# ViktorNfa/bluerov2_dynamics

Hardware: AMD Instinct MI355X
Metric: rk4_rollout_steps_per_s (higher is better)
Workload: dtype f64; 1 GPU; BASELINE config 2: 65536 trajectories/GPU x 5000 RK4 steps, thruster model, dt=0.02, iid U(-1,1) commands (splitmix64 stream 0x5EED), layout tpb, all states stored; trajectories_per_gpu=65536, horizon=5000, parallelism=1 x independent shards, no collective

## Files before the change

bluerov2_dynamics_amd/_lib.py:

```python
import ctypes
import os
import threading

import numpy as np

from . import _build

c_double_p = ctypes.POINTER(ctypes.c_double)
c_void_p = ctypes.c_void_p
i64 = ctypes.c_int64

THRUSTER_EULER, WRENCH_EULER, WRENCH_QUAT = 0, 1, 2
DI_THRUSTER_EULER, DI_WRENCH_EULER, DI_WRENCH_QUAT = 3, 4, 5
EULER, RK4 = 0, 1
LAG_PER_CALL, LAG_PER_STEP = 0, 1
LAYOUT_BTU, LAYOUT_TUB, LAYOUT_TPB = 0, 1, 2
DIST_IID_UNIFORM, DIST_AR1 = 0, 1
NX = {THRUSTER_EULER: 12, WRENCH_EULER: 12, WRENCH_QUAT: 13, DI_THRUSTER_EULER: 12, DI_WRENCH_EULER: 12, DI_WRENCH_QUAT: 13}
NU = {THRUSTER_EULER: 8, WRENCH_EULER: 6, WRENCH_QUAT: 6, DI_THRUSTER_EULER: 8, DI_WRENCH_EULER: 6, DI_WRENCH_QUAT: 6}
STATUS = {0: "BROV_OK", -1: "BROV_ERR_ARG", -2: "BROV_ERR_HIP", -3: "BROV_ERR_NOMEM", -4: "BROV_ERR_NODEVICE", -5: "BROV_ERR_COMM"}
COMM_ID_BYTES = 128


class BrovParams(ctypes.Structure):
# ... 160 lines not shown
                                       ctypes.POINTER(BrovUkf), i64, i64, ctypes.c_double] + [c_void_p] * 16 + [i64]),
    "brov_ukf_smooth_dev": (ctypes.c_int, [c_void_p, ctypes.c_int, ctypes.c_int, ctypes.c_int, i64, ctypes.POINTER(BrovParams), i64,
                                           ctypes.POINTER(BrovUkf), i64, i64, ctypes.c_double] + [c_void_p] * 16 + [i64]),
    "brov_mppi_step": (ctypes.c_int, [c_void_p, ctypes.c_int, ctypes.c_int, ctypes.c_int, i64, i64, ctypes.POINTER(BrovParams),
                                      ctypes.POINTER(BrovMppi), i64, i64, ctypes.c_double, ctypes.c_uint64, c_void_p, c_void_p, c_void_p,
                                      i64, i64, c_void_p, c_void_p, ctypes.c_int, c_void_p, c_void_p, c_void_p]),
    "brov_mppi_step_dev": (ctypes.c_int, [c_void_p, ctypes.c_int, ctypes.c_int, ctypes.c_int, i64, i64, ctypes.POINTER(BrovParams),
                                          ctypes.POINTER(BrovMppi), i64, i64, ctypes.c_double, ctypes.c_uint64, c_void_p, c_void_p,
                                          c_void_p, i64, i64, c_void_p, c_void_p, ctypes.c_int, c_void_p, c_void_p, c_void_p]),
    "edmdc_mppi_step": (ctypes.c_int, [c_void_p, ctypes.c_int, ctypes.c_int, ctypes.c_int, ctypes.c_double, c_void_p, c_void_p, c_void_p, c_void_p,
                                       c_void_p, i64, ctypes.POINTER(BrovMppi), i64, i64, ctypes.c_double, ctypes.c_uint64, c_void_p, c_void_p,
                                       i64, i64, c_void_p, c_void_p, ctypes.c_int, c_void_p, c_void_p, c_void_p, c_void_p]),
    "edmdc_mppi_step_dev": (ctypes.c_int, [c_void_p, ctypes.c_int, ctypes.c_int, ctypes.c_int, ctypes.c_double, c_void_p, c_void_p, c_void_p,
                                           c_void_p, c_void_p, i64, ctypes.POINTER(BrovMppi), i64, i64, ctypes.c_double, ctypes.c_uint64,
                                           c_void_p, c_void_p, i64, i64, c_void_p, c_void_p, ctypes.c_int, c_void_p, c_void_p, c_void_p,
                                           c_void_p]),
    "edmdc_lmpc_step": (ctypes.c_int, [c_void_p, ctypes.c_int, ctypes.c_int, ctypes.c_int, ctypes.c_double] + [c_void_p] * 6 +
                        [i64, ctypes.POINTER(BrovLmpc), i64, ctypes.c_double, c_void_p, c_void_p, i64, i64, c_void_p, c_void_p, ctypes.c_int,
                         c_void_p, c_void_p, c_void_p]),
    "edmdc_lmpc_step_dev": (ctypes.c_int, [c_void_p, ctypes.c_int, ctypes.c_int, ctypes.c_int, ctypes.c_double] + [c_void_p] * 6 +
                            [i64, ctypes.POINTER(BrovLmpc), i64, ctypes.c_double, c_void_p, c_void_p, i64, i64, c_void_p, c_void_p,
                             ctypes.c_int, c_void_p, c_void_p, c_void_p]),
    "edmdc_lmpc_block_lds": (ctypes.c_int, [i64, ctypes.POINTER(ctypes.c_int)]),
    "brov_pinc_set_weights": (ctypes.c_int, [c_void_p, c_void_p, i64]),
    "brov_pinc_forward_dev": (ctypes.c_int, [c_void_p, i64, c_void_p, c_void_p]),
    "brov_pinc_rollout": (ctypes.c_int, [c_void_p, i64, i64, ctypes.c_double, c_void_p, c_void_p, c_void_p, c_void_p, i64, c_void_p]),
    "brov_pinc_rollout_dev": (ctypes.c_int, [c_void_p, i64, i64, ctypes.c_double, c_void_p, c_void_p, c_void_p, c_void_p, i64, c_void_p]),
    "brov_pinc_window_endpoint_se": (ctypes.c_int, [c_void_p, i64, i64, ctypes.c_double, c_void_p, c_void_p, ctypes.c_int, c_void_p,
                                                    c_void_p, c_void_p, c_void_p]),
    "brov_pinc_window_endpoint_se_dev": (ctypes.c_int, [c_void_p, i64, i64, ctypes.c_double, c_void_p, c_void_p, ctypes.c_int, c_void_p,
                                                        c_void_p, c_void_p, c_void_p]),
    "brov_pinc_loss_grad_dev": (ctypes.c_int, [c_void_p, c_void_p, i64, c_void_p, c_void_p, c_void_p, ctypes.c_int, ctypes.c_int,
                                               c_void_p, c_void_p]),
    "brov_pinc_adamw_step_dev": (ctypes.c_int, [c_void_p, c_void_p, c_void_p, c_void_p, c_void_p, i64] + [ctypes.c_double] * 6 + [c_void_p]),
    "brov_pinc_train_begin": (ctypes.c_int, [c_void_p, c_void_p, i64, ctypes.POINTER(PincHyper)]),
    "brov_pinc_train_set_state": (ctypes.c_int, [c_void_p, c_void_p, c_void_p, i64]),
    "brov_pinc_train_epoch_dev": (ctypes.c_int, [c_void_p, i64, c_void_p, c_void_p, c_void_p, c_void_p, c_void_p]),
    "brov_pinc_train_get": (ctypes.c_int, [c_void_p, c_void_p, c_void_p, c_void_p, ctypes.POINTER(i64)]),
    "brov_pinc_train_end": (ctypes.c_int, [c_void_p]),
    "brov_thruster_stream": (ctypes.c_int, [c_void_p, i64, c_void_p, ctypes.c_double, c_void_p, c_void_p]),
    "brov_thruster_stream_dev": (ctypes.c_int, [c_void_p, i64, c_void_p, ctypes.c_double, c_void_p, c_void_p]),
    "brov_fill_controls_dev": (ctypes.c_int, [c_void_p, ctypes.c_int, ctypes.c_int, i64, i64, ctypes.c_int,
                                              ctypes.c_uint64, i64, i64, c_void_p, c_void_p]),
    "edmdc_lift": (ctypes.c_int, [c_void_p, i64, ctypes.c_int, ctypes.c_int, ctypes.c_double, c_void_p, c_void_p, c_void_p]),
    "edmdc_gram": (ctypes.c_int, [c_void_p, ctypes.c_int, ctypes.c_int, ctypes.c_int, ctypes.c_double, c_void_p,
                                  i64, i64, i64, i64, c_void_p, c_void_p, ctypes.c_int, c_void_p, c_void_p]),
    "edmdc_gram_dev": (ctypes.c_int, [c_void_p, ctypes.c_int, ctypes.c_int, ctypes.c_int, ctypes.c_double, c_void_p,
                                      i64, i64, i64, i64, c_void_p, c_void_p, ctypes.c_int, c_void_p, c_void_p]),
    "edmdc_gram_ragged": (ctypes.c_int, [c_void_p, ctypes.c_int, ctypes.c_int, ctypes.c_int, ctypes.c_double, c_void_p,
                                         i64, c_void_p, c_void_p, c_void_p, ctypes.c_int, c_void_p, c_void_p]),
    "edmdc_gram_ragged_dev": (ctypes.c_int, [c_void_p, ctypes.c_int, ctypes.c_int, ctypes.c_int, ctypes.c_double, c_void_p,
                                             i64, c_void_p, c_void_p, c_void_p, ctypes.c_int, c_void_p, c_void_p]),
    "edmdc_pinv_apply_ragged": (ctypes.c_int, [c_void_p, ctypes.c_int, ctypes.c_int, ctypes.c_int, ctypes.c_double, c_void_p,
                                               i64, c_void_p, c_void_p, c_void_p, c_void_p, c_void_p]),
    "edmdc_pinv_apply_ragged_dev": (ctypes.c_int, [c_void_p, ctypes.c_int, ctypes.c_int, ctypes.c_int, ctypes.c_double, c_void_p,
                                                   i64, c_void_p, c_void_p, c_void_p, c_void_p, c_void_p]),
    "brov_upload_bags": (ctypes.c_int, [c_void_p, i64, c_void_p, c_void_p, c_void_p, ctypes.c_int, c_void_p]),
    "edmdc_set_chunk_rows": (ctypes.c_int, [c_void_p, i64]),
    "edmdc_kmeans_lloyd": (ctypes.c_int, [c_void_p, i64, ctypes.c_int, ctypes.c_int, c_void_p, c_void_p, c_void_p, ctypes.c_int,
                                          ctypes.c_double, c_void_p, ctypes.POINTER(ctypes.c_double), ctypes.POINTER(ctypes.c_int)]),
    "edmdc_kmeans_lloyd_dev": (ctypes.c_int, [c_void_p, i64, ctypes.c_int, ctypes.c_int, c_void_p, i64, c_void_p, c_void_p, ctypes.c_int,
                                              ctypes.c_double, c_void_p, ctypes.POINTER(ctypes.c_double), ctypes.POINTER(ctypes.c_int)]),
    "edmdc_kmeanspp_dev": (ctypes.c_int, [c_void_p, i64, ctypes.c_int, ctypes.c_int, c_void_p, i64, c_void_p, i64, ctypes.c_int, c_void_p,
                                          c_void_p, c_void_p]),
    "edmdc_multistep_se": (ctypes.c_int, [c_void_p, ctypes.c_int, ctypes.c_int, ctypes.c_int, ctypes.c_double, c_void_p,
                                          c_void_p, c_void_p, i64, i64, c_void_p, c_void_p, c_void_p, c_void_p]),
    "edmdc_multistep_se_linear": (ctypes.c_int, [c_void_p, ctypes.c_int, ctypes.c_int, ctypes.c_int, ctypes.c_double, c_void_p,
                                                 c_void_p, c_void_p, i64, i64, c_void_p, c_void_p, c_void_p, c_void_p]),
    "edmdc_simulate": (ctypes.c_int, [c_void_p, ctypes.c_int, ctypes.c_int, ctypes.c_int, ctypes.c_double, c_void_p,
                                      c_void_p, c_void_p, i64, i64, c_void_p, c_void_p, c_void_p]),
    "edmdc_pinv_apply": (ctypes.c_int, [c_void_p, ctypes.c_int, ctypes.c_int, ctypes.c_int, ctypes.c_double, c_void_p,
                                        i64, i64, i64, i64, c_void_p, c_void_p, c_void_p, c_void_p]),
    "edmdc_pinv_apply_dev": (ctypes.c_int, [c_void_p, ctypes.c_int, ctypes.c_int, ctypes.c_int, ctypes.c_double, c_void_p,
                                            i64, i64, i64, i64, c_void_p, c_void_p, c_void_p, c_void_p]),
    "edmdc_gram_decomposition": (ctypes.c_int, [ctypes.c_int, ctypes.c_int, ctypes.c_int, ctypes.POINTER(ctypes.c_int), ctypes.POINTER(ctypes.c_int)]),
    "edmdc_gtg_decomposition": (ctypes.c_int, [ctypes.c_int, ctypes.c_int, ctypes.c_int, ctypes.POINTER(ctypes.c_int), ctypes.POINTER(ctypes.c_int)]),
    "edmdc_apply_decomposition": (ctypes.c_int, [ctypes.c_int, ctypes.c_int, ctypes.c_int] + [ctypes.POINTER(ctypes.c_int)] * 4),
    "edmdc_set_apply_variant": (ctypes.c_int, [c_void_p, ctypes.c_int]),
    "edmdc_lift_cache": (ctypes.c_int, [c_void_p, c_void_p, ctypes.c_size_t]),
    "edmdc_set_kmeans_variant": (ctypes.c_int, [c_void_p, ctypes.c_int]),
    "edmdc_set_kmeans_bounds_rate": (ctypes.c_int, [c_void_p, ctypes.c_double]),
    "brov_experiments_build": (ctypes.c_int, []),
    "brov_set_rollout_variant": (ctypes.c_int, [c_void_p, ctypes.c_int]),
    "edmdc_set_kmeans_far_select": (ctypes.c_int, [c_void_p, c_void_p, c_void_p]),
    "edmdc_kmeans_relocations": (ctypes.c_int, [c_void_p]),
    "edmdc_kmeans_loop_info": (ctypes.c_int, [c_void_p, ctypes.POINTER(ctypes.c_int)]),
    "edmdc_far_select_numpy": (ctypes.c_int, [c_void_p, i64, ctypes.c_int, c_void_p]),
    "edmdc_set_kmeans_allreduce": (ctypes.c_int, [c_void_p, c_void_p, c_void_p]),
    "edmdc_set_kmeans_shard": (ctypes.c_int, [c_void_p, ctypes.c_int, ctypes.c_int, i64, i64]),
    "brov_comm_available": (ctypes.c_int, []),
    "brov_comm_unique_id": (ctypes.c_int, [c_void_p]),
    "brov_comm_init_rank": (ctypes.c_int, [ctypes.c_int, c_void_p, ctypes.c_int, ctypes.c_int, ctypes.POINTER(c_void_p)]),
    "brov_comm_destroy": (None, [c_void_p]),
    "brov_comm_nranks": (ctypes.c_int, [c_void_p]),
    "brov_comm_rank": (ctypes.c_int, [c_void_p]),
    "brov_comm_last_error": (ctypes.c_char_p, [c_void_p]),
    "edmdc_gram_allreduce_dev": (ctypes.c_int, [c_void_p, c_void_p, i64, c_void_p, i64, c_void_p]),
    "brov_comm_allreduce_words": (ctypes.c_int, [c_void_p, c_void_p, i64, ctypes.c_int, c_void_p]),
    "edmdc_kmeans_use_comm": (ctypes.c_int, [c_void_p, c_void_p]),
}


def library_path():
    return _build.LIB


hip_runtime = None


def _one_hip_runtime():
    import sys
    if "torch" in sys.modules:
        return "torch (imported by the caller)"
    mode = os.environ.get("BROV2_TORCH", "auto").strip().lower()
    if mode in ("1", "import", "yes", "true"):
        try:
            import torch
            return "torch (imported by load_library: BROV2_TORCH=1)"
        except ImportError:
            return "system (BROV2_TORCH=1 but torch is not installed)"
    if mode in ("0", "no", "never", "false"):
        return "system (BROV2_TORCH=0)"
    try:
        import importlib.util
        spec = importlib.util.find_spec("torch")
    except (ImportError, ValueError):
        spec = None
    if spec is not None and spec.origin:
        cand = os.path.join(os.path.dirname(spec.origin), "lib", "libamdhip64.so")
        if os.path.exists(cand):
            try:
                ctypes.CDLL(cand, mode=ctypes.RTLD_GLOBAL)
                return "torch's libamdhip64.so preloaded (torch itself not imported)"
            except OSError:
                pass
    return "system"


def load_library():
    global _lib, hip_runtime
    with _lib_lock:
        if _lib is not None:
            return _lib
        path = library_path()
        if not os.path.exists(path):
            raise BrovError(
                f"{path} is missing: build it with `python -c 'import __graft_entry__ as g; g.build()'` "
                "(hipcc --offload-arch=gfx950). There is no CPU fallback.")
        hip_runtime = _one_hip_runtime()
        lib = ctypes.CDLL(path)
        for name, (res, args) in SIGNATURES.items():
            fn = getattr(lib, name)
            fn.restype = res
            fn.argtypes = args
        if lib.brov_abi_version() != 1:
            raise BrovError("libbrov2.so ABI version mismatch")
        _lib = lib
        return lib


def default_params() -> BrovParams:
    p = BrovParams()
    load_library().brov_default_params(ctypes.byref(p))
    return p


# ... 33 lines not shown

class Context:

    def __init__(self, device: int = 0):
        self.lib = load_library()
        h = c_void_p()
        rc = self.lib.brov_create(int(device), ctypes.byref(h))
        if rc != 0:
            raise BrovError(f"brov_create(device={device}) failed: {STATUS.get(rc, rc)} -- a gfx950 GPU is required, "
                            "there is no CPU fallback")
        self.h = h
        self.device = int(device)
        self._stream = 0
        self._allreduce_cb = None
        self.check(self.lib.edmdc_set_kmeans_far_select(self.h, ctypes.cast(_NUMPY_FAR_SELECT, c_void_p), None), "edmdc_set_kmeans_far_select")

    @property
    def arch(self) -> str:
        buf = ctypes.create_string_buffer(64)
        self.check(self.lib.brov_device_arch(self.h, buf, 64), "brov_device_arch")
        return buf.value.decode()

    @property
    def xcd_round_robin(self) -> int:
        return int(self.lib.brov_xcd_round_robin(self.h))

    def close(self):
        if getattr(self, "h", None):
            self.lib.brov_destroy(self.h)
            self.h = None

    def __del__(self):
        try:
            self.close()
        except Exception:
            pass

    def check(self, rc, what=""):
        if rc != 0:
            msg = self.lib.brov_last_error(self.h)
            raise BrovError(f"{what}: {STATUS.get(rc, rc)}: {msg.decode() if msg else ''}")

    def get_params(self) -> BrovParams:
        p = BrovParams()
        self.check(self.lib.brov_get_params(self.h, ctypes.byref(p)), "brov_get_params")
        return p

    def set_params(self, p: BrovParams):
        self.check(self.lib.brov_set_params(self.h, ctypes.byref(p)), "brov_set_params")

    def set_stream(self, stream_handle):
        stream_handle = int(stream_handle or 0)
        if stream_handle != self._stream:
            self.check(self.lib.brov_set_stream(self.h, c_void_p(stream_handle)), "brov_set_stream")
            self._stream = stream_handle

    def use_torch_stream(self):
        import torch
        self.set_stream(torch.cuda.current_stream(self.device).cuda_stream)

    def use_null_stream(self):
        self.set_stream(0)

    def set_di_gains(self, K_lin, K_ang):
        K_lin, K_ang = as_f64(K_lin), as_f64(K_ang)
        assert K_lin.shape == K_ang.shape and K_lin.shape[1] == 3
        self.check(self.lib.brov_set_di_gains(self.h, int(K_lin.shape[0]), K_lin.ctypes.data, K_ang.ctypes.data), "brov_set_di_gains")

    def set_btu_staging(self, mode: int):
        self.check(self.lib.brov_set_btu_staging(self.h, int(mode)), "brov_set_btu_staging")

    def lift_cache(self, device_ptr, nbytes: int = 0):
        self.check(self.lib.edmdc_lift_cache(self.h, c_void_p(device_ptr or 0), int(nbytes if device_ptr else 0)), "edmdc_lift_cache")

    def set_kmeans_variant(self, variant: int):
        self.check(self.lib.edmdc_set_kmeans_variant(self.h, int(variant)), "edmdc_set_kmeans_variant")

    def set_kmeans_bounds_rate(self, rate: float):
        self.check(self.lib.edmdc_set_kmeans_bounds_rate(self.h, float(rate)), "edmdc_set_kmeans_bounds_rate")

    def set_rollout_variant(self, variant: int):
        self.check(self.lib.brov_set_rollout_variant(self.h, int(variant)), "brov_set_rollout_variant")

    def set_kmeans_far_select(self, numpy_rule: bool):
        fn = ctypes.cast(_NUMPY_FAR_SELECT, c_void_p) if numpy_rule else None
        self.check(self.lib.edmdc_set_kmeans_far_select(self.h, fn, None), "edmdc_set_kmeans_far_select")

    def kmeans_relocations(self) -> int:
        return int(self.lib.edmdc_kmeans_relocations(self.h))

    def kmeans_loop_info(self) -> dict:
        v = (ctypes.c_int * 4)()
        self.check(self.lib.edmdc_kmeans_loop_info(self.h, v), "edmdc_kmeans_loop_info")
        return dict(relocations=v[0], resorts=v[1], first_resort_iteration=v[2], list_form_e_steps=v[3])

    def set_kmeans_allreduce(self, fn):
        if fn is None:
            self._allreduce_cb = None
            self.check(self.lib.edmdc_set_kmeans_allreduce(self.h, None, None), "edmdc_set_kmeans_allreduce")
            return

        def tramp(_user, ptr, count, op):
            try:
                fn(int(ptr), int(count), int(op))
                return 0
            except Exception:
                import traceback
                traceback.print_exc()
                return 1
        self._allreduce_cb = ALLREDUCE_FN(tramp)
        self.check(self.lib.edmdc_set_kmeans_allreduce(self.h, ctypes.cast(self._allreduce_cb, c_void_p), None), "edmdc_set_kmeans_allreduce")

    def set_kmeans_shard(self, rank: int = 0, world: int = 1, row_offset: int = 0, n_global: int = 0):
        self.check(self.lib.edmdc_set_kmeans_shard(self.h, int(rank), int(world), int(row_offset), int(n_global)), "edmdc_set_kmeans_shard")

    def kmeans_use_comm(self, comm):
        self.check(self.lib.edmdc_kmeans_use_comm(self.h, comm.h if comm is not None else None), "edmdc_kmeans_use_comm")

    def set_apply_variant(self, variant: int):
        self.check(self.lib.edmdc_set_apply_variant(self.h, int(variant)), "edmdc_set_apply_variant")

    def sync(self):
        self.check(self.lib.brov_sync(self.h), "brov_sync")

    def set_timing(self, on: bool):
        self.check(self.lib.brov_set_timing(self.h, int(bool(on))), "brov_set_timing")
        self.timing = bool(on)

    def last_kernel_ms(self) -> float:
        ms = ctypes.c_float(0.0)
        self.check(self.lib.brov_last_kernel_ms(self.h, ctypes.byref(ms)), "brov_last_kernel_ms")
        return float(ms.value)


_default = {}
_default_lock = threading.Lock()


def default_context(device: int = None) -> Context:
    if device is None:
        device = int(os.environ.get("BROV2_DEVICE", os.environ.get("LOCAL_RANK", "0")))
    ctx = _default.get(device)
    if ctx is None:
        with _default_lock:
            ctx = _default.get(device)
            if ctx is None:
                ctx = _default[device] = Context(device)
    return ctx


def warm_up(device: int = None, block: bool = False):
    def work():
        try:
            default_context(device)
        except Exception:
            pass
    if block:
        return default_context(device)
    t = threading.Thread(target=work, name="brov2-warm-up", daemon=True)
    t.start()
    return t


class Comm:

    def __init__(self, device: int, unique_id: bytes, nranks: int, rank: int):
# ... 48 lines not shown
```

bluerov2_dynamics_amd/csrc/brov2_fast.h:

```cpp
#pragma once
#include "brov2_device.h"

namespace brov {

struct FastParams {
    double E[12];
    double da[6], db[6];
    double G[5];
    double lc[4][3];
    double ld[4];
    double Tm[6][8];
    double minv[6];
    double poly[5];
    double A1[9], b1[3];
    double A4[9], b4[3];
    double Ob[9];
    double al4[3];
    double Aw4[9], bw4[3];
    double g1[3];
    double XY[4];
    double cur[3];
    int has_current;
    int has_xy;
    int tm_dense;
    int obs_bad;
};

typedef const FastParams __attribute__((address_space(4)))* CFP;
__device__ __forceinline__ CFP as_constant(const FastParams* g) { return (CFP)(unsigned long long)g; }

template <bool RES>
struct HotConstsT {
    static constexpr bool RESIDENT = RES;
    double E[12], db[6];
    double da[6], G[5], ld[4], al4[3];
    double tk[2];
};
typedef HotConstsT<false> HotConsts;
typedef HotConstsT<true> HotConstsResident;

#ifndef BROV_CLAMP_BRANCH
#define BROV_CLAMP_BRANCH 1
#endif
#ifndef BROV_PSI_FRAME
#define BROV_PSI_FRAME 1
#endif
#define BROV_PIN_V(x) asm volatile("" : "+v"(x))
#define BROV_PIN_S(x) asm volatile("" : "+s"(x))
#define BROV_FORM_HERE(r) asm volatile("" : "+v"(r))
#define BROV_SC(h, p, f) (HC::RESIDENT ? (h).f : (p)->f)

template <bool RES>
__device__ __forceinline__ void load_hot(CFP pp, HotConstsT<RES>& h) {
    const auto& p = *pp;
#pragma unroll
    for (int i = 0; i < 12; ++i) { h.E[i] = p.E[i]; BROV_PIN_V(h.E[i]); }
#pragma unroll
    for (int i = 0; i < 6; ++i) { h.db[i] = p.db[i]; BROV_PIN_V(h.db[i]); }
    if constexpr (RES) {
#pragma unroll
        for (int i = 0; i < 6; ++i) { h.da[i] = p.da[i]; BROV_PIN_S(h.da[i]); }
#pragma unroll
        for (int i = 0; i < 5; ++i) { h.G[i] = p.G[i]; BROV_PIN_S(h.G[i]); }
#pragma unroll
        for (int i = 0; i < 4; ++i) { h.ld[i] = p.ld[i]; BROV_PIN_S(h.ld[i]); }
#pragma unroll
        for (int i = 0; i < 3; ++i) { h.al4[i] = p.al4[i]; BROV_PIN_S(h.al4[i]); }
        h.tk[0] = -1.98412698298579493134e-04; BROV_PIN_V(h.tk[0]);
        h.tk[1] = 2.48015872894767294178e-05;  BROV_PIN_V(h.tk[1]);
    }
}

template <bool GENERIC, class HC>
__device__ __forceinline__ const double* trig_consts(const HC& h) {
    if constexpr (HC::RESIDENT && !GENERIC) return h.tk; else return nullptr;
}

__device__ __forceinline__ CFP relaunder(CFP p) {
    asm volatile("" : "+s"(p));
    return p;
}

__device__ __forceinline__ void sincos_fast(double x, double& s, double& c, const double2* __restrict__ qt, const double* kv = nullptr) {
    const double S7 = kv ? kv[0] : -1.98412698298579493134e-04, C8 = kv ? kv[1] : 2.48015872894767294178e-05;
    const double kf = rint(x * 6.36619772367581382433e-01);
    double r = fma(-kf, 1.57079632673412561417e+00, x);
    r = fma(-kf, 6.07710050630396597660e-11, r);
    r = fma(-kf, 2.02226624879595063154e-21, r);
    const int q = (int)kf;
    const double z = r * r;
    double ps = fma(z, 1.58969099521155010221e-10, -2.50507602534068634195e-08);
    ps = fma(z, ps, 2.75573137070700676789e-06);
    ps = fma(z, ps, S7);
    ps = fma(z, ps, 8.33333333332248946124e-03);
    ps = fma(z, ps, -1.66666666666666324348e-01);
    const double sr = fma(z * r, ps, r);
    double pc = fma(z, -1.13596475577881948265e-11, 2.08757232129817482790e-09);
    pc = fma(z, pc, -2.75573143513906633035e-07);
    pc = fma(z, pc, C8);
    pc = fma(z, pc, -1.38888888888741095749e-03);
    pc = fma(z, pc, 4.16666666666666019037e-02);
    const double cr = fma(z * z, pc, fma(-0.5, z, 1.0));
    const double2 t = qt[q & 3];
    s = fma(cr, t.y, sr * t.x);
    c = fma(-sr, t.y, cr * t.x);
}

__device__ __forceinline__ void init_quadrant_table(double2* qt) {
    if (threadIdx.x < 4) {
        const int q = threadIdx.x;
        qt[q] = make_double2(q == 0 ? 1.0 : (q == 2 ? -1.0 : 0.0), q == 1 ? 1.0 : (q == 3 ? -1.0 : 0.0));
    }
}

struct Trig { double sphi, cphi, sth, cth, spsi, cpsi; };

__device__ __forceinline__ void trig_full(const double* ang, Trig& t, const double2* __restrict__ qt, const double* kv = nullptr) {
    sincos_fast(ang[0], t.sphi, t.cphi, qt, kv);
    sincos_fast(ang[1], t.sth, t.cth, qt, kv);
    sincos_fast(ang[2], t.spsi, t.cpsi, qt, kv);
}

template <bool SHORT = false, bool LEAN = false>
__device__ __forceinline__ void trig_delta(const Trig& b, double d[3], Trig& t, double* dpsi = nullptr, const double* kv = nullptr) {
    constexpr int K0 = SHORT ? 4 : 3;
    const double S7 = kv ? kv[0] : -1.98412698298579493134e-04, C8 = kv ? kv[1] : 2.48015872894767294178e-05;
    double dcopy[3] = {d[0], d[1], d[2]};
    double* dd = LEAN ? d : dcopy;
    int k = 0;
    const double m = fmax(fmax(fabs(d[0]), fabs(d[1])), fabs(d[2]));
    const bool far = !(m <= (SHORT ? 0.0625 : 0.125));
    if (far) {
        double mf = m;
        if constexpr (LEAN) asm volatile("; trig_delta range extension, rare" : "+v"(mf));
        int e;
        (void)frexp(mf, &e);
        k = e + K0;
        double sc = ldexp(1.0, -k);
        if (!(mf < 0x1p37)) { sc = __builtin_nan(""); k = 0; }
#pragma unroll
        for (int i = 0; i < 3; ++i) dd[i] *= sc;
    }
    double sd[3], cm[3];
#pragma unroll
    for (int i = 0; i < 3; ++i) {
        const double z = dd[i] * dd[i];
        double ps, pc;
        if constexpr (SHORT) {
            ps = fma(z, S7, 8.33333333332248946124e-03);
            pc = fma(z, C8, -1.38888888888741095749e-03);
        } else {
            ps = fma(z, 2.75573137070700676789e-06, S7);
            ps = fma(z, ps, 8.33333333332248946124e-03);
            pc = fma(z, -2.75573143513906633035e-07, C8);
            pc = fma(z, pc, -1.38888888888741095749e-03);
        }
        ps = fma(z, ps, -1.66666666666666324348e-01);
        sd[i] = fma(z * dd[i], ps, dd[i]);
        pc = fma(z, pc, 4.16666666666666019037e-02);
        pc = fma(z, pc, -0.5);
        cm[i] = z * pc;
    }
    auto doubling = [&](int n) {
        for (int j = 0; j < n; ++j) {
#pragma unroll
            for (int i = 0; i < 3; ++i) {
                const double t2 = sd[i] + sd[i];
                const double s2 = fma(t2, cm[i], t2);
                cm[i] = -(t2 * sd[i]);
                sd[i] = s2;
            }
        }
    };
    if constexpr (LEAN) {
        if (far) {
            double mf = m;
            asm volatile("; trig_delta doubling, rare" : "+v"(mf));
            int e;
            (void)frexp(mf, &e);
            doubling((mf < 0x1p37) ? e + K0 : 0);
        }
    } else doubling(k);
    t.sphi = fma(b.cphi, sd[0], fma(b.sphi, cm[0], b.sphi)); t.cphi = fma(-b.sphi, sd[0], fma(b.cphi, cm[0], b.cphi));
    t.sth = fma(b.cth, sd[1], fma(b.sth, cm[1], b.sth));     t.cth = fma(-b.sth, sd[1], fma(b.cth, cm[1], b.cth));
    t.spsi = fma(b.cpsi, sd[2], fma(b.spsi, cm[2], b.spsi)); t.cpsi = fma(-b.spsi, sd[2], fma(b.cpsi, cm[2], b.cpsi));
    if (dpsi) { dpsi[0] = sd[2]; dpsi[1] = cm[2]; }
}

#ifndef BROV_TRIG_SHORT
#define BROV_TRIG_SHORT 1
#endif
__device__ __forceinline__ double recip_fast(double x) {
    double y = __builtin_amdgcn_rcp(x);
    double e = fma(-x, y, 1.0);
    y = fma(y, e, y);
    e = fma(-x, y, 1.0);
    return fma(y, e, y);
}

template <bool GENERIC, class HC>
__device__ __forceinline__ void nu_dot_fast(const HC& h, CFP p, const double R[9], const double nu[6],
                                            const double a[6], double sth, double ctsp, double ctcp, double out[6]) {
    const double u = nu[0], v = nu[1], w = nu[2], pp = nu[3], q = nu[4], r = nu[5];
    double nr0 = u, nr1 = v, nr2 = w;
    if (GENERIC && p->has_current) {
        nr0 -= fma(R[6], p->cur[2], fma(R[3], p->cur[1], R[0] * p->cur[0]));
        nr1 -= fma(R[7], p->cur[2], fma(R[4], p->cur[1], R[1] * p->cur[0]));
        nr2 -= fma(R[8], p->cur[2], fma(R[5], p->cur[1], R[2] * p->cur[0]));
    }
    double o0 = fma(-h.E[0], w * q, a[0]);  o0 = fma(h.E[1], v * r, o0);
    double o1 = fma(-h.E[2], u * r, a[1]);  o1 = fma(h.E[3], w * pp, o1);
    double o2 = fma(-h.E[4], v * pp, a[2]); o2 = fma(h.E[5], u * q, o2);
    double o3 = fma(-h.E[6], v * w, a[3]);  o3 = fma(-h.E[7], q * r, o3);
    double o4 = fma(-h.E[8], u * w, a[4]);  o4 = fma(-h.E[9], pp * r, o4);
    double o5 = fma(-h.E[10], u * v, a[5]); o5 = fma(-h.E[11], pp * q, o5);
    o0 = fma(-fma(h.db[0], fabs(nr0), BROV_SC(h, p, da[0])), nr0, o0);
    o1 = fma(-fma(h.db[1], fabs(nr1), BROV_SC(h, p, da[1])), nr1, o1);
    o2 = fma(-fma(h.db[2], fabs(nr2), BROV_SC(h, p, da[2])), nr2, o2);
    o3 = fma(-fma(h.db[3], fabs(pp), BROV_SC(h, p, da[3])), pp, o3);
    o4 = fma(-fma(h.db[4], fabs(q), BROV_SC(h, p, da[4])), q, o4);
    o5 = fma(-fma(h.db[5], fabs(r), BROV_SC(h, p, da[5])), r, o5);
    o0 = fma(-BROV_SC(h, p, G[0]), sth, o0);
    o1 = fma(BROV_SC(h, p, G[1]), ctsp, o1);
    o2 = fma(BROV_SC(h, p, G[2]), ctcp, o2);
    o3 = fma(BROV_SC(h, p, G[3]), ctsp, o3);
    o4 = fma(BROV_SC(h, p, G[4]), sth, o4);
    if (GENERIC && p->has_xy) {
        o3 = fma(-p->XY[0], ctcp, o3);
        o4 = fma(p->XY[1], ctcp, o4);
        o5 = fma(-p->XY[2], ctsp, o5);
        o5 = fma(-p->XY[3], sth, o5);
    }
    out[0] = o0; out[1] = o1; out[2] = o2; out[3] = o3; out[4] = o4; out[5] = o5;
}

template <bool GENERIC, class HC, bool PFRAME = false>
__device__ __forceinline__ void rhs_fast_euler(const HC& h, CFP p, const double x[12], const double a[6], double xd[12], const Trig& tg) {
    const double sphi = tg.sphi, cphi = tg.cphi, sth = tg.sth, cth = tg.cth, spsi = tg.spsi, cpsi = tg.cpsi;
    const double* nu = x + 6;
    const double ctsp = cth * sphi, ctcp = cth * cphi;
    if constexpr (GENERIC) {
        double R[9];
        const double ss = sth * sphi, sc = sth * cphi;
        R[0] = cpsi * cth; R[1] = fma(cpsi, ss, -(spsi * cphi)); R[2] = fma(cpsi, sc, spsi * sphi);
        R[3] = spsi * cth; R[4] = fma(spsi, ss, cpsi * cphi);    R[5] = fma(spsi, sc, -(cpsi * sphi));
        R[6] = -sth;       R[7] = ctsp;                          R[8] = ctcp;
        nu_dot_fast<true>(h, p, R, nu, a, sth, ctsp, ctcp, xd + 6);
#pragma unroll
        for (int i = 0; i < 3; ++i) xd[i] = fma(R[3 * i + 2], nu[2], fma(R[3 * i + 1], nu[1], R[3 * i] * nu[0]));
    } else {
        nu_dot_fast<false>(h, p, nullptr, nu, a, sth, ctsp, ctcp, xd + 6);
        const double y1 = fma(cphi, nu[1], -(sphi * nu[2])), z1 = fma(sphi, nu[1], cphi * nu[2]);
        const double x2 = fma(cth, nu[0], sth * z1), z2 = fma(cth, z1, -(sth * nu[0]));
        if constexpr (PFRAME) { xd[0] = x2; xd[1] = y1; }
        else {
            xd[0] = fma(cpsi, x2, -(spsi * y1));
            xd[1] = fma(spsi, x2, cpsi * y1);
        }
        xd[2] = z2;
    }
#if BROV_CLAMP_BRANCH
    double ic = recip_fast(cth);
    if (__builtin_amdgcn_ballot_w64(fabs(cth) < 1e-7) != 0) {
        asm volatile("; cos(theta) clamp, rare" ::: "memory");
        if (fabs(cth) < 1e-7) ic = recip_fast(1e-7 * ((cth > 0.0) - (cth < 0.0)));
    }
#else
    double cc = cth;
    if (fabs(cc) < 1e-7) cc = 1e-7 * ((cc > 0.0) - (cc < 0.0));
    const double ic = recip_fast(cc);
#endif
    const double m = fma(sphi, nu[4], cphi * nu[5]);
    xd[3] = fma(sth * ic, m, nu[3]);
    xd[4] = fma(cphi, nu[4], -(sphi * nu[5]));
    xd[5] = ic * m;
}

template <bool GENERIC, class HC>
__device__ __forceinline__ void rhs_fast_quat(const HC& h, CFP p, const double x[13], const double a[6], double xd[13]) {
    double q[4] = {x[3], x[4], x[5], x[6]};
    quat_normalize(q);
    const double qw = q[0], qx = q[1], qy = q[2], qz = q[3];
    double R[9];
    R[0] = 1.0 - 2.0 * fma(qy, qy, qz * qz); R[1] = 2.0 * fma(qx, qy, -(qz * qw));    R[2] = 2.0 * fma(qx, qz, qy * qw);
    R[3] = 2.0 * fma(qx, qy, qz * qw);       R[4] = 1.0 - 2.0 * fma(qx, qx, qz * qz); R[5] = 2.0 * fma(qy, qz, -(qx * qw));
    R[6] = 2.0 * fma(qx, qz, -(qy * qw));    R[7] = 2.0 * fma(qy, qz, qx * qw);       R[8] = 1.0 - 2.0 * fma(qx, qx, qy * qy);
    const double* nu = x + 7;
    nu_dot_fast<GENERIC>(h, p, R, nu, a, -R[6], R[7], R[8], xd + 7);
#pragma unroll
    for (int i = 0; i < 3; ++i) xd[i] = fma(R[3 * i + 2], nu[2], fma(R[3 * i + 1], nu[1], R[3 * i] * nu[0]));
    const double wx = nu[3], wy = nu[4], wz = nu[5];
    xd[3] = 0.5 * (-(qx * wx) - qy * wy - qz * wz);
    xd[4] = 0.5 * (qw * wx + qy * wz - qz * wy);
    xd[5] = 0.5 * (qw * wy - qx * wz + qz * wx);
    xd[6] = 0.5 * (qw * wz + qx * wy - qy * wx);
}

__device__ __forceinline__ void rhs_di_euler(const double x[12], const double a[6], double xd[12], const Trig& tg) {
    const double sphi = tg.sphi, cphi = tg.cphi, sth = tg.sth, cth = tg.cth, spsi = tg.spsi, cpsi = tg.cpsi;
    const double* v = x + 6;
    const double y1 = fma(cphi, v[1], -(sphi * v[2])), z1 = fma(sphi, v[1], cphi * v[2]);
    const double x2 = fma(cth, v[0], sth * z1);
    xd[0] = fma(cpsi, x2, -(spsi * y1));
    xd[1] = fma(spsi, x2, cpsi * y1);
    xd[2] = fma(cth, z1, -(sth * v[0]));
#pragma unroll
    for (int i = 0; i < 3; ++i) xd[3 + i] = x[9 + i];
#pragma unroll
    for (int i = 0; i < 6; ++i) xd[6 + i] = a[i];
}
__device__ __forceinline__ void rhs_di_quat(const double x[13], const double a[6], double xd[13]) {
    double q[4] = {x[3], x[4], x[5], x[6]};
    quat_normalize(q);
    const double qw = q[0], qx = q[1], qy = q[2], qz = q[3];
    const double R0 = 1.0 - 2.0 * fma(qy, qy, qz * qz), R1 = 2.0 * fma(qx, qy, -(qz * qw)), R2 = 2.0 * fma(qx, qz, qy * qw);
    const double R3 = 2.0 * fma(qx, qy, qz * qw), R4 = 1.0 - 2.0 * fma(qx, qx, qz * qz), R5 = 2.0 * fma(qy, qz, -(qx * qw));
    const double R6 = 2.0 * fma(qx, qz, -(qy * qw)), R7 = 2.0 * fma(qy, qz, qx * qw), R8 = 1.0 - 2.0 * fma(qx, qx, qy * qy);
    const double* v = x + 7;
    xd[0] = fma(R2, v[2], fma(R1, v[1], R0 * v[0]));
    xd[1] = fma(R5, v[2], fma(R4, v[1], R3 * v[0]));
    xd[2] = fma(R8, v[2], fma(R7, v[1], R6 * v[0]));
    const double wx = x[10], wy = x[11], wz = x[12];
    xd[3] = 0.5 * (-(qx * wx) - qy * wy - qz * wz);
    xd[4] = 0.5 * (qw * wx + qy * wz - qz * wy);
    xd[5] = 0.5 * (qw * wy - qx * wz + qz * wx);
    xd[6] = 0.5 * (qw * wz + qx * wy - qy * wx);
#pragma unroll
    for (int i = 0; i < 6; ++i) xd[7 + i] = a[i];
}

template <int MODEL, bool GENERIC, class HC, bool PFRAME = false>
__device__ __forceinline__ void rhs_fast(const HC& h, CFP p, const double* x, const double a[6], double* xd, const Trig& tg) {
    if constexpr (MODEL == MODEL_DI_WRENCH_QUAT) rhs_di_quat(x, a, xd);
    else if constexpr (model_is_di(MODEL)) rhs_di_euler(x, a, xd, tg);
    else if constexpr (MODEL == MODEL_WRENCH_QUAT) rhs_fast_quat<GENERIC>(h, p, x, a, xd);
    else rhs_fast_euler<GENERIC, HC, PFRAME>(h, p, x, a, xd, tg);
}

struct LagZ {
    double z[6][3];
    __device__ __forceinline__ void zero() {
#pragma unroll
        for (int k = 0; k < 6; ++k) { z[k][0] = 0.0; z[k][1] = 0.0; z[k][2] = 0.0; }
    }
    __device__ __forceinline__ void from_thrusters(CFP p, const double X[8][3]) {
#pragma unroll
        for (int k = 0; k < 6; ++k)
#pragma unroll
            for (int j = 0; j < 3; ++j) {
                double a = p->Tm[k][0] * X[0][j];
#pragma unroll
                for (int i = 1; i < 8; ++i) a = fma(p->Tm[k][i], X[i][j], a);
                z[k][j] = a;
            }
    }
    __device__ __forceinline__ void accel_after(CFP p, int s, const double acmd[6], double a[6]) const {
        const double c0 = p->lc[s - 1][0], c1 = p->lc[s - 1][1], c2 = p->lc[s - 1][2], d = p->ld[s - 1];
#pragma unroll
        for (int k = 0; k < 6; ++k) a[k] = fma(c2, z[k][2], fma(c1, z[k][1], fma(c0, z[k][0], d * acmd[k])));
    }
    __device__ __forceinline__ void to_observer(CFP p) {
#pragma unroll
        for (int k = 0; k < 6; ++k) {
            const double a0 = z[k][0], a1 = z[k][1], a2 = z[k][2];
            z[k][0] = fma(p->Ob[2], a2, fma(p->Ob[1], a1, p->Ob[0] * a0));
            z[k][1] = fma(p->Ob[5], a2, fma(p->Ob[4], a1, p->Ob[3] * a0));
            z[k][2] = fma(p->Ob[8], a2, fma(p->Ob[7], a1, p->Ob[6] * a0));
        }
    }
    template <class HC>
    __device__ __forceinline__ void obs_accel_after(const HC& h, CFP p, int s, const double acmd[6], double a[6]) const {
        if (s <= 3) {
            const double d = BROV_SC(h, p, ld[s - 1]);
#pragma unroll
            for (int k = 0; k < 6; ++k) a[k] = fma(d, acmd[k], z[k][s - 1]);
        } else {
            const double c0 = BROV_SC(h, p, al4[0]), c1 = BROV_SC(h, p, al4[1]), c2 = BROV_SC(h, p, al4[2]), d = BROV_SC(h, p, ld[3]);
#pragma unroll
            for (int k = 0; k < 6; ++k) a[k] = fma(c2, z[k][2], fma(c1, z[k][1], fma(c0, z[k][0], d * acmd[k])));
        }
    }
    __device__ __forceinline__ void obs_advance1(CFP p, const double acmd[6]) {
        const double c0 = p->al4[0], c1 = p->al4[1], c2 = p->al4[2], g0 = p->g1[0], g1 = p->g1[1], g2 = p->g1[2];
#pragma unroll
        for (int k = 0; k < 6; ++k) {
            const double a0 = z[k][0], a1 = z[k][1], a2 = z[k][2];
            z[k][0] = fma(g0, acmd[k], a1);
            z[k][1] = fma(g1, acmd[k], a2);
            z[k][2] = fma(c2, a2, fma(c1, a1, fma(c0, a0, g2 * acmd[k])));
        }
    }
    __device__ __forceinline__ void advance(const double __attribute__((address_space(4)))* A, const double __attribute__((address_space(4)))* b, const double acmd[6]) {
#pragma unroll
        for (int k = 0; k < 6; ++k) {
            const double a0 = z[k][0], a1 = z[k][1], a2 = z[k][2];
            const double q0 = fma(A[1], a1, fma(A[0], a0, b[0] * acmd[k]));
            const double q1 = fma(A[4], a1, fma(A[3], a0, b[1] * acmd[k]));
            const double q2 = fma(A[7], a1, fma(A[6], a0, b[2] * acmd[k]));
            double n0 = a0, n1 = a1, n2 = a2;
            asm("v_fma_f64 %0, %1, %2, %3" : "+v"(n0) : "s"(A[2]), "v"(a2), "v"(q0), "v"(q1), "v"(q2));
            asm("v_fma_f64 %0, %1, %2, %3" : "+v"(n1) : "s"(A[5]), "v"(a2), "v"(q1), "v"(q0), "v"(q2));
            asm("v_fma_f64 %0, %1, %0, %2" : "+v"(n2) : "s"(A[8]), "v"(q2), "v"(n0), "v"(n1));
            z[k][0] = n0; z[k][1] = n1; z[k][2] = n2;
        }
    }
};

__device__ __forceinline__ void advance_thrusters(const double __attribute__((address_space(4)))* A, const double __attribute__((address_space(4)))* b, const double fcmd[8], double X[8][3]) {
#pragma unroll
    for (int i = 0; i < 8; ++i) {
        const double a0 = X[i][0], a1 = X[i][1], a2 = X[i][2];
        X[i][0] = fma(A[2], a2, fma(A[1], a1, fma(A[0], a0, b[0] * fcmd[i])));
        X[i][1] = fma(A[5], a2, fma(A[4], a1, fma(A[3], a0, b[1] * fcmd[i])));
        X[i][2] = fma(A[8], a2, fma(A[7], a1, fma(A[6], a0, b[2] * fcmd[i])));
    }
}

template <int MODEL, bool SPARSE>
__device__ __forceinline__ void command_accel(CFP p, const double* u, double fcmd[8], double acmd[6]) {
    if constexpr (MODEL == MODEL_THRUSTER_EULER) {
#pragma unroll
        for (int i = 0; i < 8; ++i) {
            const double V = u[i], V2 = V * V;
            double hh = fma(V2, p->poly[4], p->poly[3]);
            hh = fma(V2, hh, p->poly[2]);
            hh = fma(V2, hh, p->poly[1]);
            hh = fma(V2, hh, p->poly[0]);
            fcmd[i] = V * hh;
        }
        if constexpr (SPARSE) {
#pragma unroll
            for (int k = 0; k < 6; ++k) {
                const int i0 = (k == 2) ? 4 : 0, i1 = (k == 3 || k == 4) ? 8 : (k == 2 ? 8 : 4);
                double a = p->Tm[k][i0] * fcmd[i0];
#pragma unroll
                for (int i = i0 + 1; i < i1; ++i) a = fma(p->Tm[k][i], fcmd[i], a);
                acmd[k] = a;
            }
        } else {
#pragma unroll
            for (int k = 0; k < 6; ++k) {
                double a = p->Tm[k][0] * fcmd[0];
#pragma unroll
                for (int i = 1; i < 8; ++i) a = fma(p->Tm[k][i], fcmd[i], a);
                acmd[k] = a;
            }
        }
    } else if constexpr (model_is_di(MODEL)) {
        constexpr int NU = Dims<MODEL>::NU;
#pragma unroll
        for (int k = 0; k < 6; ++k) {
            double a = p->Tm[k][0] * u[0];
#pragma unroll
            for (int i = 1; i < NU; ++i) a = fma(p->Tm[k][i], u[i], a);
            acmd[k] = a;
        }
    } else {
#pragma unroll
        for (int k = 0; k < 6; ++k) acmd[k] = p->minv[k] * u[k];
    }
}

template <int MODEL, int INTEG, bool GENERIC, class HC, class AccelFn>
__device__ __forceinline__ void integrate_fast(const HC& h, CFP p, double dt, double* x, AccelFn&& accel,
                                               const double2* qt, Trig* carry, bool refresh) {
    constexpr int NX = Dims<MODEL>::NX;
    constexpr bool ANG = !model_is_quat(MODEL);
    constexpr bool LEAN = HC::RESIDENT && !GENERIC;
    double a[6];
    Trig tb, ts;
    const bool CARRY = ANG && carry != nullptr;
    if constexpr (ANG) {
        if (!CARRY || refresh) trig_full(x + 3, tb, qt, trig_consts<GENERIC>(h));
        else tb = *carry;
    }
    double dang[3];
    if constexpr (INTEG == INTEG_EULER) {
        double k[NX];
        accel(1, a);
        rhs_fast<MODEL, GENERIC>(h, p, x, a, k, tb);
        if (CARRY) {
#pragma unroll
            for (int i = 0; i < NX; ++i) {
                if (i >= 3 && i < 6) {
                    if constexpr (LEAN) {
#pragma clang fp contract(off)
                        dang[i - 3] = dt * k[i]; x[i] += dang[i - 3]; BROV_FORM_HERE(x[i]);
                    } else { dang[i - 3] = dt * k[i]; x[i] += dang[i - 3]; }
                } else x[i] = fma(dt, k[i], x[i]);
            }
        } else {
#pragma unroll
            for (int i = 0; i < NX; ++i) x[i] = fma(dt, k[i], x[i]);
        }
    } else {
        double k[NX], xn[NX], xs[NX], dl[3];
        const double h2 = 0.5 * dt, h6 = dt / 6.0, h3 = dt / 3.0;
        constexpr bool PSIF = BROV_PSI_FRAME && ANG && !GENERIC && !model_is_di(MODEL);
        double dps[2] = {0.0, 0.0};
        auto stage_state = [&](double c, auto HALF) {
#pragma unroll
            for (int i = 0; i < NX; ++i) {
                if (ANG && i >= 3 && i < 6) dl[i - 3] = c * k[i];
                else xs[i] = fma(c, k[i], x[i]);
            }
            if constexpr (ANG) trig_delta<BROV_TRIG_SHORT && decltype(HALF)::value, LEAN>(tb, dl, ts, PSIF ? dps : nullptr, trig_consts<GENERIC>(h));
        };
        auto add_turned = [&](double w) {
            const double r0 = fma(dps[1], k[0], fma(-dps[0], k[1], k[0])), r1 = fma(dps[0], k[0], fma(dps[1], k[1], k[1]));
            xn[0] = fma(w, r0, xn[0]);
            xn[1] = fma(w, r1, xn[1]);
        };
        accel(1, a);
        rhs_fast<MODEL, GENERIC, HC, PSIF>(h, p, x, a, k, tb);
#pragma unroll
        for (int i = 0; i < NX; ++i) xn[i] = ((CARRY && i >= 3 && i < 6) || (PSIF && i < 2)) ? h6 * k[i] : fma(h6, k[i], x[i]);
        stage_state(h2, std::true_type{});
        accel(2, a);
        rhs_fast<MODEL, GENERIC, HC, PSIF>(h, p, xs, a, k, ts);
#pragma unroll
        for (int i = PSIF ? 2 : 0; i < NX; ++i) xn[i] = fma(h3, k[i], xn[i]);
        if constexpr (PSIF) add_turned(h3);
        stage_state(h2, std::true_type{});
        accel(3, a);
        rhs_fast<MODEL, GENERIC, HC, PSIF>(h, p, xs, a, k, ts);
#pragma unroll
        for (int i = PSIF ? 2 : 0; i < NX; ++i) xn[i] = fma(h3, k[i], xn[i]);
        if constexpr (PSIF) add_turned(h3);
        stage_state(dt, std::false_type{});
        accel(4, a);
        rhs_fast<MODEL, GENERIC, HC, PSIF>(h, p, xs, a, k, ts);
        if constexpr (PSIF) {
            add_turned(h6);
            x[0] = fma(tb.cpsi, xn[0], fma(-tb.spsi, xn[1], x[0]));
            x[1] = fma(tb.spsi, xn[0], fma(tb.cpsi, xn[1], x[1]));
        }
        if (CARRY) {
#pragma unroll
            for (int i = PSIF ? 2 : 0; i < NX; ++i) {
                if (i >= 3 && i < 6) { dang[i - 3] = fma(h6, k[i], xn[i]); x[i] += dang[i - 3]; if constexpr (LEAN) BROV_FORM_HERE(x[i]); }
                else x[i] = fma(h6, k[i], xn[i]);
            }
        } else {
#pragma unroll
            for (int i = PSIF ? 2 : 0; i < NX; ++i) x[i] = fma(h6, k[i], xn[i]);
        }
    }
    if constexpr (ANG) { if (CARRY) trig_delta<false, LEAN>(tb, dang, *carry, nullptr, trig_consts<GENERIC>(h)); }
    if constexpr (model_is_quat(MODEL)) quat_normalize(x + 3);
}

template <int INTEG, int LAGMODE, bool TRACK, bool GENERIC>
__device__ __forceinline__ void lag_step_advance(CFP pl, LagZ& lz, const double fcmd[8], const double acmd[6], double X[8][3]) {
    constexpr bool OBS = !GENERIC;
    if constexpr (INTEG == INTEG_RK4 && LAGMODE == 0) {
        if constexpr (OBS) lz.advance(pl->Aw4, pl->bw4, acmd); else lz.advance(pl->A4, pl->b4, acmd);
        if constexpr (TRACK) advance_thrusters(pl->A4, pl->b4, fcmd, X);
    } else {
        if constexpr (OBS) lz.obs_advance1(pl, acmd); else lz.advance(pl->A1, pl->b1, acmd);
        if constexpr (TRACK) advance_thrusters(pl->A1, pl->b1, fcmd, X);
    }
}
template <int LAGMODE, bool GENERIC, class HC>
__device__ __forceinline__ void lag_stage_accel(const HC& h, CFP p, const LagZ& lz, int s, const double acmd[6], double a[6]) {
    const int se = LAGMODE == 0 ? s : 1;
    if constexpr (!GENERIC) lz.obs_accel_after(h, p, se, acmd, a); else lz.accel_after(p, se, acmd, a);
}

template <int MODEL, int INTEG, int LAGMODE, bool TRACK, bool GENERIC, class HC>
__device__ __forceinline__ void step_fast(const HC& h, CFP p0, double dt, double* x, const double* u,
                                          LagZ& lz, double X[8][3], const double2* qt, Trig* carry = nullptr, bool refresh = true) {
    constexpr bool THR = (MODEL == MODEL_THRUSTER_EULER);
    CFP p = relaunder(p0);
    double fcmd[8], acmd[6];
    if constexpr (MODEL == MODEL_DI_WRENCH_QUAT) quat_normalize(x + 3);
    command_accel<MODEL, !GENERIC>(p, u, fcmd, acmd);
    integrate_fast<MODEL, INTEG, GENERIC>(h, p, dt, x, [&](int s, double* a) {
        if constexpr (THR) lag_stage_accel<LAGMODE, GENERIC>(h, p, lz, s, acmd, a);
        else {
#pragma unroll
            for (int k = 0; k < 6; ++k) a[k] = acmd[k];
        }
    }, qt, carry, refresh);
    if constexpr (THR) lag_step_advance<INTEG, LAGMODE, TRACK, GENERIC>(relaunder(p0), lz, fcmd, acmd, X);
}

}
```

bluerov2_dynamics_amd/csrc/brov2_kernels.h:

```cpp
#pragma once
#include <hip/hip_runtime.h>
#include <stdint.h>
#include "brov2_device.h"
#include "brov2_fast.h"

namespace brov {

hipError_t launch_rhs(hipStream_t st, const DevParams& p, int model, int64_t B, const double* x, const double* u,
                      double* lag, double* xd, unsigned long long* done = nullptr, unsigned long long seq = 0);
hipError_t launch_thruster_forces(hipStream_t st, const DevParams& p, int64_t B, const double* u, double* lag, double* tau,
                                  unsigned long long* done = nullptr, unsigned long long seq = 0);
hipError_t launch_rollout(hipStream_t st, const FastParams* d_fp, int model, int integ, int lag_mode, int layout, int64_t B,
                          int64_t T, double dt, const double* x0, const double* U, double* lag, double* traj,
                          int64_t stride, double* xT, int btu_staging);
hipError_t launch_rollout_pop(hipStream_t st, const FastParams* d_fp, int model, int integ, int lag_mode, int P, int per_candidate,
                              int64_t B, int64_t T, double dt, const double* x0, const double* U, double* lag, double* traj,
                              int64_t stride, double* xT);
struct FeedbackRec {
    double K[8][12], Ki[8][6];
    double u_min[8], u_max[8];
    double z_max[6];
    int32_t hold, pad;
};
struct FeedbackArgs {
    const FastParams* fp;
    const FeedbackRec* fb;
    int fb_per_candidate, per_candidate;
    int64_t B, T, ref_rows, stride;
    double dt;
    const double *x0, *u_ff, *ref;
    double *lag, *z, *traj, *xT, *u_applied, *metrics;
};
hipError_t launch_rollout_feedback(hipStream_t st, int model, int integ, int lag_mode, int P, const FeedbackArgs& a);
struct UkfRec {
    double q[12], r[12];
    double c, wc0, wi, pad;
};
struct UkfArgs {
    const FastParams* fp;
    const UkfRec* rec;
    int rec_per_candidate, pad;
    int64_t B, T;
    double dt;
    const double *x0, *P0, *U, *Y;
    double *lag, *xf, *pstd, *innov, *xT, *PT, *info;
    double *tape, *nrows;
    int64_t Bs;
};
constexpr int UKF_TAPE = 312;
int ukf_waves_per_block();
hipError_t launch_ukf_filter(hipStream_t st, int model, int integ, int lag_mode, int P, const UkfArgs& a);
struct UkfRtsArgs {
    int64_t B, T, Bs;
    const double *xf, *tape, *nrows, *xsT, *PsT;
    double *xs, *pstd, *Ps, *Ps0, *sinfo;
};
hipError_t launch_ukf_rts(hipStream_t st, int P, const UkfRtsArgs& a);
struct MppiRec {
    double q[12], qf[12];
    double r[8], sigma[8];
    double u_min[8], u_max[8];
    double lambda, gamma;
    int32_t hold, pad;
};
struct MppiArgs {
    const FastParams* fp;
    const MppiRec* rec;
    int per_problem, shift;
    int64_t K, H, M, ref_total, ref_row0;
    double dt;
    uint64_t seed;
    const double *x, *lag, *ref, *eps;
    double *U_nom, *U_old, *u_apply, *cost, *info;
};
hipError_t launch_mppi_step(hipStream_t st, int model, int integ, int lag_mode, int64_t B, const MppiArgs& a);
hipError_t launch_mppi_update(hipStream_t st, int nu, int64_t B, const MppiArgs& a);
constexpr int KOOPMAN_MPPI_MAX_K = 1024;
constexpr int KOOPMAN_MPPI_MAX_MNU = 312;
struct KoopmanMppiArgs {
    MppiArgs m;
    int n, r, k;
    double gamma;
    const double *C, *P, *Gc;
    double *F, *pred;
};
int koopman_mppi_block(int64_t K, int64_t mnu);
hipError_t launch_koopman_mppi_step(hipStream_t st, int64_t B, const KoopmanMppiArgs& a);
hipError_t launch_koopman_free(hipStream_t st, int64_t B, const KoopmanMppiArgs& a);
struct LmpcRec {
    double q[13], qf[13];
    double r[8];
    double u_min[8], u_max[8];
    double rho, tol;
    int32_t hold, iters;
};
struct KoopmanQpArgs {
    KoopmanMppiArgs f;
// ... 206 lines not shown
```

bluerov2_dynamics_amd/csrc/capi.hip:

```cpp
#include <hip/hip_runtime.h>
#include <algorithm>
#include <cmath>
#include <cstdio>
#include <cstdlib>
#include <cstring>
#include <new>
#include <string>
#include <ctime>
#include <thread>
#include <unordered_map>
#include <utility>
#include <vector>

#include "../../include/brov2.h"
#include "brov2_kernels.h"

using namespace brov;

struct brov_ctx {
    int device = 0;
    hipStream_t stream = nullptr;
    brov_params params;
    std::string err;
    bool timing = false;
    hipEvent_t ev0 = nullptr, ev1 = nullptr;
    bool timed = false;
    char* scratch = nullptr;
    size_t scratch_cap = 0;
    char* ukf_tape = nullptr;
    size_t ukf_tape_cap = 0;
    bool dp_valid = false;
    double dp_dt = 0.0;
    DevParams dp;
    FastParams fp;
    FastParams* d_fp = nullptr;
    FastParams* d_fp_di = nullptr;
    bool di_set = false;
    float* d_pinc = nullptr;
    bool pinc_set = false;
    float* d_pinc_part = nullptr;
    int pinc_part_cap = 0;
    float* d_train = nullptr;
    bool train_on = false;
    int64_t train_step = 0;
    brov_pinc_hyper train_hyper = {};
    int btu_staging = 0;
    int single_lane = 0;
    int64_t chunk_rows = (int64_t)1 << 20;
    char* lift_cache = nullptr;
    size_t lift_cache_cap = 0;
    bool lift_cache_valid = false;
    struct LiftKey { const void *X, *U, *C; int n, r, k; double gamma; int64_t nbags, L, xs, us, chunk; uint64_t bag_hash; } lift_key = {};
    int kmeans_variant = 0;
    double km_bounds_rate = 0.03;
    int apply_variant = 0;
    void* d_tasks[3] = {nullptr, nullptr, nullptr};
    EdmdcShape task_shape[3] = {};
    int ntasks[3] = {0, 0, 0};
    double* d_partial = nullptr;
    size_t partial_cap = 0;
    size_t tasks_cap[3] = {0, 0, 0};
    hipEvent_t ev_handover = nullptr;
    hipStream_t side[3] = {nullptr, nullptr, nullptr};
    hipEvent_t ev_fork = nullptr, ev_join[3] = {nullptr, nullptr, nullptr};
    double* h_io = nullptr;
    double* d_io = nullptr;
    unsigned long long io_seq = 0;
    std::vector<std::pair<void*, size_t>> pool;
    std::unordered_map<void*, size_t> live;
    size_t pool_bytes = 0;
    char* h_stage[2] = {nullptr, nullptr};
    hipEvent_t ev_stage[2] = {nullptr, nullptr};
    int upload_threads = 0;
    double* h_stats = nullptr;
    double km_seq = 0.0;
    double* d_stats_map = nullptr;
    brov_far_select_fn far_select = nullptr;
    void* far_select_user = nullptr;
    brov_allreduce_fn km_allreduce = nullptr;
    void* km_allreduce_user = nullptr;
    brov_comm* km_comm = nullptr;
    long long km_row_offset = 0;
    int km_rank = 0, km_world = 1;
    long long km_n_global = 0;
    int kmeans_relocations = 0;
    int km_info[4] = {0, 0, 0, 0};
    int prop_groups = 2;
    int xcd_round_robin = -1;
    char arch[64] = {0};
};

enum : int {
    KMV_FULL_SCAN = 1,
    KMV_UNSORTED = 2,
    KMV_NO_BOUNDS = 4,
    KMV_PUBLIC = 7,
    KMV_PP_UNSCREENED = 8,
    KMV_MASK_FILTER = 16,
    KMV_PP_SHARD_KERNELS = 32,
    KMV_PK_STANDALONE = 64,
    KMV_NO_SCREENING = 128,
    KMV_SCALAR_RECORDS = 256,
#ifdef BROV2_EXPERIMENTS
    KMV_ACCEPTED = 511,
#else
    KMV_ACCEPTED = KMV_PUBLIC,
#endif
};

static hipError_t h2d_copy(brov_ctx* c, void* dst, const void* src, size_t bytes);
static hipError_t d2h_copy(brov_ctx* c, void* dst, const void* src, size_t bytes);

namespace {

int fail(brov_ctx* c, int code, const std::string& msg) {
    if (c) c->err = msg;
    return code;
}
int hip_fail(brov_ctx* c, hipError_t e, const char* what) {
    return fail(c, e == hipErrorOutOfMemory ? BROV_ERR_NOMEM : BROV_ERR_HIP, std::string(what) + ": " + hipGetErrorString(e));
}
#define HIPCK(ctx, call) do { hipError_t e__ = (call); if (e__ != hipSuccess) return hip_fail((ctx), e__, #call); } while (0)

struct DeviceGuard {
    int prev = -1;
    bool switched = false;
    explicit DeviceGuard(const brov_ctx* c) {
        if (hipGetDevice(&prev) != hipSuccess) prev = -1;
        if (prev != c->device) { (void)hipSetDevice(c->device); switched = true; }
    }
// ... 899 lines not shown
    DeviceGuard g(c);
    const DevParams* dp;
    int rc = get_dp(c, dt, &dp);
    if (rc) return rc;
    if (B <= SMALL_B) {
        rc = ensure_io(c);
        if (rc) return rc;
        const size_t ou = 0, ol = ou + B * 8, ot = ol + B * 24;
        std::memcpy(c->h_io + ou, u, B * 8 * 8);
        std::memcpy(c->h_io + ol, lag_io, B * 24 * 8);
        const bool spin = !c->timing;
        const unsigned long long seq = ++c->io_seq;
        {
            CallTimer t(c);
            HIPCK(c, launch_thruster_forces(c->stream, *dp, B, c->d_io + ou, c->d_io + ol, c->d_io + ot,
                                            spin ? reinterpret_cast<unsigned long long*>(c->d_io + IO_FLAGS) : nullptr, seq));
        }
        if (spin) { rc = wait_flags(c, B, seq, "brov_thruster_forces"); if (rc) return rc; }
        else HIPCK(c, hipStreamSynchronize(c->stream));
        std::memcpy(tau, c->h_io + ot, B * 6 * 8);
        std::memcpy(lag_io, c->h_io + ol, B * 24 * 8);
        return BROV_OK;
    }
    Arena a(c, true);
    double *du, *dtau, *dl;
    rc = a.lay("brov_thruster_forces", [&] {
        du = a.in(u, B * 8);
        dtau = a.out(tau, B * 6);
        dl = a.inout(lag_io, B * 24);
    });
    if (rc) return rc;
    {
        CallTimer t(c);
        HIPCK(c, launch_thruster_forces(c->stream, *dp, B, du, dl, dtau));
    }
    return a.finish();
}

static int rollout_args_ok(brov_ctx* c, int model, int integ, int lag_mode, int layout, int64_t B, int64_t T, int64_t stride,
                           const void* x0, const void* U, const void* traj) {
    if (!c) return BROV_ERR_ARG;
    if (!model_ok(model) || (integ != BROV_EULER && integ != BROV_RK4) || (lag_mode != BROV_LAG_PER_CALL && lag_mode != BROV_LAG_PER_STEP) ||
        (layout != BROV_LAYOUT_BTU && layout != BROV_LAYOUT_TUB && layout != BROV_LAYOUT_TPB) || B < 0 || T < 0)
        return fail(c, BROV_ERR_ARG, "brov_rollout: bad enum or negative size");
    if (B && (!x0 || (T && !U))) return fail(c, BROV_ERR_ARG, "brov_rollout: NULL input");
    if (traj && stride < 1) return fail(c, BROV_ERR_ARG, "brov_rollout: traj_stride must be >= 1");
    return BROV_OK;
}

int brov_set_di_gains(brov_ctx* c, int nu, const double* K_lin, const double* K_ang) {
    if (!c || (nu != 6 && nu != 8) || !K_lin || !K_ang) return fail(c, BROV_ERR_ARG, "brov_set_di_gains: nu must be 6 or 8");
    DeviceGuard g(c);
    FastParams f;
    std::memset(&f, 0, sizeof f);
    for (int i = 0; i < nu; ++i)
        for (int k = 0; k < 3; ++k) { f.Tm[k][i] = K_lin[3 * i + k]; f.Tm[3 + k][i] = K_ang[3 * i + k]; }
    if (!c->d_fp_di) HIPCK(c, hipMalloc((void**)&c->d_fp_di, sizeof(FastParams)));
    HIPCK(c, h2d_copy(c, c->d_fp_di, &f, sizeof f));
    HIPCK(c, hipStreamSynchronize(c->stream));
    c->di_set = true;
    return BROV_OK;
}

int brov_set_btu_staging(brov_ctx* c, int mode) {
    if (!c || mode < 0 || mode > 2) return fail(c, BROV_ERR_ARG, "brov_set_btu_staging: mode must be 0, 1 or 2");
    c->btu_staging = mode;
    return BROV_OK;
}

int brov_rollout_dev(brov_ctx* c, int model, int integ, int lag_mode, int layout, int64_t B, int64_t T, double dt,
                     const double* d_x0, const double* d_U, double* d_lag_io, double* d_traj, int64_t stride, double* d_xT) {
    int rc = rollout_args_ok(c, model, integ, lag_mode, layout, B, T, stride, d_x0, d_U, d_traj);
    if (rc) return rc;
    if (B == 0) return BROV_OK;
    DeviceGuard g(c);
    const DevParams* dp;
    rc = get_dp(c, dt, &dp);
    if (rc) return rc;
    if (model_is_di_h(model) && !c->di_set) return fail(c, BROV_ERR_ARG, "double-integrator model: call brov_set_di_gains first");
    CallTimer t(c);
    HIPCK(c, launch_rollout(c->stream, model_is_di_h(model) ? c->d_fp_di : c->d_fp, model, integ, lag_mode, layout, B, T, dt, d_x0, d_U,
                            d_lag_io, d_traj, d_traj ? stride : 1, d_xT,
                            c->btu_staging | ((c->fp.has_current || c->fp.has_xy || c->fp.tm_dense || c->fp.obs_bad) ? 4 : 0) |
                                (c->single_lane ? 8 : 0)));
    return BROV_OK;
}

int brov_rollout(brov_ctx* c, int model, int integ, int lag_mode, int layout, int64_t B, int64_t T, double dt,
                 const double* x0, const double* U, double* lag_io, double* traj, int64_t stride, double* xT) {
    int rc = rollout_args_ok(c, model, integ, lag_mode, layout, B, T, stride, x0, U, traj);
    if (rc) return rc;
    if (B == 0) return BROV_OK;
    DeviceGuard g(c);
    const int nx = NX(model), nu = NU(model);
    const bool lag = lag_io && model == BROV_THRUSTER_EULER;
    const int64_t rows = traj ? T / stride + 1 : 0;
    const int nuw = layout == BROV_LAYOUT_TPB ? (nu + 1) / 2 * 2 : nu;
    const int nxw = layout == BROV_LAYOUT_TPB ? (nx + 1) / 2 * 2 : nx;
    Arena a(c, true);
    double *dx0, *dU, *dxT, *dl, *dtr;
    rc = a.lay("brov_rollout", [&] {
        dx0 = a.in(x0, B * nx);
        dU = a.in(U, (size_t)B * T * nuw);
        dxT = a.out(xT, B * nx);
        dl = lag ? a.inout(lag_io, B * 24) : nullptr;
        dtr = traj ? a.out(traj, (size_t)B * rows * nxw) : nullptr;
    });
    if (rc) return rc;
    rc = brov_rollout_dev(c, model, integ, lag_mode, layout, B, T, dt, dx0, dU, dl, dtr, stride, dxT);
    if (rc) return rc;
    return a.finish();
}

static void lag_window_phi(const DevParams& dp, int64_t samples, double Phi[9]) {
    double R[9] = {1, 0, 0, 0, 1, 0, 0, 0, 1}, Bq[9];
    std::memcpy(Bq, dp.lag_A[0], sizeof Bq);
    while (samples > 0) {
        if (samples & 1) matmul(3, R, Bq, R);
        matmul(3, Bq, Bq, Bq);
        samples >>= 1;
    }
    std::memcpy(Phi, R, sizeof R);
}

static int64_t window_chunks(int64_t nwin) { return (nwin + window_scan_chunk() - 1) / window_scan_chunk(); }
static void lag_window_phi_pair(const DevParams& dp, int64_t samples, double out18[18]) {
    lag_window_phi(dp, samples, out18);
    lag_window_phi(dp, samples * window_scan_chunk(), out18 + 9);
}

static int derive_candidates(brov_ctx* c, int integ, int P, const brov_params* params, int64_t H, double dt, bool scan,
                             std::vector<FastParams>& fp, std::vector<double>& phi) {
    if (!(dt > 0.0) || !std::isfinite(dt)) return fail(c, BROV_ERR_ARG, "dt must be finite and > 0");
    fp.resize((size_t)P);
    phi.resize(scan ? (size_t)P * 18 : 0);
    for (int j = 0; j < P; ++j) {
        const brov_params& p = params[j];
        const double md[6] = {p.m - p.added_mass[0], p.m - p.added_mass[1], p.m - p.added_mass[2],
                              p.Ix - p.added_mass[3], p.Iy - p.added_mass[4], p.Iz - p.added_mass[5]};
        for (int i = 0; i < 6; ++i)
            if (!(md[i] != 0.0) || !std::isfinite(md[i])) return fail(c, BROV_ERR_ARG, "candidate " + std::to_string(j) + ": singular mass matrix");
        DevParams dp;
        if (!derive(p, dt, dp)) return fail(c, BROV_ERR_ARG, "thruster-lag discretisation failed (singular Pade system)");
        derive_fast(p, dp, fp[j]);
        if (scan) lag_window_phi_pair(dp, H * (integ == BROV_RK4 ? 4 : 1), &phi[(size_t)j * 18]);
    }
    return BROV_OK;
}

struct WindowBags {
    int64_t nbags = 0, rows = 0, nwin = 0;
    std::vector<int64_t> tab;
};
static int window_bags(brov_ctx* c, int64_t nbags, const int64_t* off, int64_t H, WindowBags* wb, const char* who) {
    if (nbags < 0 || !off) return fail(c, BROV_ERR_ARG, std::string(who) + ": bad bag list (nbags >= 0, bag_offsets [nbags + 1])");
    if (off[0] != 0) return fail(c, BROV_ERR_ARG, std::string(who) + ": bag_offsets[0] must be 0");
    wb->tab.assign((size_t)(2 * (nbags + 1)), 0);
    int64_t* wpre = wb->tab.data();
    for (int64_t b = 0; b < nbags; ++b) {
        const int64_t L = off[b + 1] - off[b];
        if (L < 0) return fail(c, BROV_ERR_ARG, std::string(who) + ": bag_offsets must not decrease");
        wpre[b + 1] = wpre[b] + (L > H ? L - H : 0);
    }
    std::copy(off, off + nbags + 1, wpre + nbags + 1);
    wb->nbags = nbags;
    wb->rows = off[nbags];
    wb->nwin = wpre[nbags];
// ... 1276 lines not shown
    int64_t ci = 0;
    for (int64_t r0 = 0; r0 < total_pairs_rows; r0 += chunk, ++ci) {
        const int64_t npairs = (total_pairs_rows - r0 < chunk) ? (total_pairs_rows - r0) : chunk;
        const int64_t rows_lift = (npairs + 3) / 4 * 4 + 1;
        double* z = caching ? reinterpret_cast<double*>(c->lift_cache + (size_t)ci * slot) : dZ;
        double* w = caching ? z + (size_t)(chunk + 8) * s.width : dw;
        HIPCK(c, launch_lift_rows_total(c->stream, s, gamma, d_C, r0, rows_lift, total_rows, L, xs, us, d_X, d_U, z, w, pf));
        HIPCK(c, launch_gram_chunk_tasks(c->stream, s, c->ntasks[mode], c->d_tasks[mode], npairs, z, z, w, c->d_partial, first ? 0 : 1));
        first = 0;
    }
    if (caching) {
        c->lift_key = {d_X, d_U, d_C, n, r, k, gamma, bl.nbags, L, xs, us, chunk, bl.hash};
        c->lift_cache_valid = true;
    }
    HIPCK(c, launch_gram_finish_tasks(c->stream, s, c->ntasks[mode], c->d_tasks[mode], c->d_partial, accumulate, d_GtG, d_GtY));
    return BROV_OK;
}

int edmdc_gram_dev(brov_ctx* c, int n, int r, int k, double gamma, const double* d_C, int64_t nbags, int64_t L,
                   int64_t xs, int64_t us, const double* d_X, const double* d_U, int accumulate, double* d_GtG, double* d_GtY) {
    int rc = edmdc_shape_ok(c, n, r, k);
    if (rc) return rc;
    if (nbags < 0 || L < 0 || !d_C || !d_GtG || (nbags && L && (!d_X || (r && !d_U))) || (nbags > 1 && (xs < L + 1 || us < L)))
        return fail(c, BROV_ERR_ARG, "edmdc_gram_dev: bad argument");
    BagLayout bl;
    bag_layout_uniform(nbags, L, xs, us, &bl);
    return gram_core(c, n, r, k, gamma, d_C, bl, d_X, d_U, accumulate, d_GtG, d_GtY);
}

int edmdc_gram_ragged_dev(brov_ctx* c, int n, int r, int k, double gamma, const double* d_C, int64_t nbags, const int64_t* bag_offsets,
                          const double* d_X, const double* d_U, int accumulate, double* d_GtG, double* d_GtY) {
    int rc = edmdc_shape_ok(c, n, r, k);
    if (rc) return rc;
    if (!d_C || !d_GtG) return fail(c, BROV_ERR_ARG, "edmdc_gram_ragged_dev: bad argument");
    BagLayout bl;
    rc = bag_layout_ragged(c, nbags, bag_offsets, &bl, "edmdc_gram_ragged_dev");
    if (rc) return rc;
    if (bl.total_rows > 1 && (!d_X || (r && !d_U))) return fail(c, BROV_ERR_ARG, "edmdc_gram_ragged_dev: bad argument");
    return gram_core(c, n, r, k, gamma, d_C, bl, d_X, d_U, accumulate, d_GtG, d_GtY);
}

int edmdc_gram_decomposition(int n, int r, int k, int* ntasks, int* nslabs) {
    if (!edmdc_shape_supported(n, r, k)) return BROV_ERR_ARG;
    (void)gram_partial_doubles(edmdc_shape(n, r, k), 0, ntasks, nslabs);
    return BROV_OK;
}

int edmdc_gtg_decomposition(int n, int r, int k, int* ntasks, int* nslabs) {
    if (!edmdc_shape_supported(n, r, k)) return BROV_ERR_ARG;
    (void)gram_partial_doubles(edmdc_shape(n, r, k), 2, ntasks, nslabs);
    return BROV_OK;
}

int edmdc_apply_decomposition(int n, int r, int k, int* wrows_items_per_192_rows, int* wrows_tiles_wanted, int* wty_tasks, int* wty_slabs) {
    if (!edmdc_shape_supported(n, r, k)) return BROV_ERR_ARG;
    const EdmdcShape s = edmdc_shape(n, r, k);
    wrows_decomposition(s, wrows_items_per_192_rows, wrows_tiles_wanted);
    (void)gram_partial_doubles(s, 1, wty_tasks, wty_slabs);
    return BROV_OK;
}

int edmdc_lift_cache(brov_ctx* c, void* d_buffer, size_t bytes) {
    if (!c || (d_buffer && (reinterpret_cast<uintptr_t>(d_buffer) & 15))) return fail(c, BROV_ERR_ARG, "edmdc_lift_cache: buffer must be 16-byte aligned");
    c->lift_cache = d_buffer ? static_cast<char*>(d_buffer) : nullptr;
    c->lift_cache_cap = d_buffer ? bytes : 0;
    c->lift_cache_valid = false;
    return BROV_OK;
}

int edmdc_set_kmeans_variant(brov_ctx* c, int variant) {
    if (!c || variant < 0 || (variant & ~KMV_ACCEPTED) != 0 || (variant & 3) == 3)
        return fail(c, BROV_ERR_ARG, "edmdc_set_kmeans_variant: variant must be 0, 1 (full scan) or 2 (no sorted order), optionally + 4 (distance bounds off)");
    c->kmeans_variant = variant;
    return BROV_OK;
}
int edmdc_set_kmeans_bounds_rate(brov_ctx* c, double rate) {
    if (!c || !(rate >= 0.0) || rate > 1.0) return fail(c, BROV_ERR_ARG, "edmdc_set_kmeans_bounds_rate: rate must lie in [0, 1]");
    c->km_bounds_rate = rate;
    return BROV_OK;
}
int brov_set_rollout_variant(brov_ctx* c, int variant) {
    if (!c || variant < 0 || variant > 1) return fail(c, BROV_ERR_ARG, "brov_set_rollout_variant: variant must be 0 or 1");
    c->single_lane = variant;
    return BROV_OK;
}
int brov_experiments_build(void) {
#ifdef BROV2_EXPERIMENTS
    return 1;
#else
    return 0;
#endif
}

int edmdc_set_kmeans_far_select(brov_ctx* c, brov_far_select_fn fn, void* user) {
    if (!c) return BROV_ERR_ARG;
    c->far_select = fn;
    c->far_select_user = user;
    return BROV_OK;
}
int edmdc_kmeans_relocations(brov_ctx* c) { return c ? c->kmeans_relocations : 0; }
int edmdc_kmeans_loop_info(brov_ctx* c, int info[4]) {
    if (!c || !info) return BROV_ERR_ARG;
    info[0] = c->kmeans_relocations; info[1] = c->km_info[1]; info[2] = c->km_info[2]; info[3] = c->km_info[3];
    return BROV_OK;
}
static void far_select_default(const double* dist, int64_t N, int n_empty, int64_t* out);
int edmdc_far_select_numpy(const double* distances, int64_t N, int n_empty, int64_t* far_rows_out) {
    if (!distances || !far_rows_out || N < 1 || n_empty < 1 || n_empty > N) return BROV_ERR_ARG;
    far_select_default(distances, N, n_empty, far_rows_out);
    return BROV_OK;
}
int edmdc_set_kmeans_allreduce(brov_ctx* c, brov_allreduce_fn fn, void* user) {
    if (!c) return BROV_ERR_ARG;
    c->km_allreduce = fn;
    c->km_allreduce_user = user;
    return BROV_OK;
}

static int km_allreduce_through_comm(void* user, void* d_buf, int64_t count, int op) {
    brov_ctx* c = static_cast<brov_ctx*>(user);
    return brov_comm_allreduce_words(c->km_comm, d_buf, count, op, c->stream);
}
int edmdc_set_kmeans_shard(brov_ctx* c, int rank, int world, int64_t row_offset, int64_t n_global) {
    if (!c || world < 1 || rank < 0 || rank >= world || row_offset < 0 || row_offset >= (1ll << 61) || n_global < 0)
        return fail(c, BROV_ERR_ARG, "edmdc_set_kmeans_shard: bad argument");
    c->km_rank = rank;
    c->km_world = world;
    c->km_row_offset = row_offset;
    c->km_n_global = n_global;
    return BROV_OK;
}
int edmdc_kmeans_use_comm(brov_ctx* c, brov_comm* comm) {
    if (!c) return BROV_ERR_ARG;
    c->km_comm = comm;
    c->km_allreduce = comm ? km_allreduce_through_comm : nullptr;
    c->km_allreduce_user = comm ? c : nullptr;
    return BROV_OK;
}

int edmdc_set_apply_variant(brov_ctx* c, int variant) {
    if (!c || variant < 0 || variant > 1) return fail(c, BROV_ERR_ARG, "edmdc_set_apply_variant: variant must be 0 or 1");
    c->apply_variant = variant;
    return BROV_OK;
}

static int apply_core(brov_ctx* c, int n, int r, int k, double gamma, const double* d_C, const BagLayout& bl,
                      const double* d_X, const double* d_U, const double* P_host, double* d_M) {
    int rc = BROV_OK;
    DeviceGuard g(c);
    const EdmdcShape s = edmdc_shape(n, r, k);
    rc = ensure_tasks(c, s, 1);
    if (rc) return rc;
    const int64_t nbags = bl.nbags, L = bl.L, xs = bl.xs, us = bl.us;
    const int64_t total_rows = bl.total_rows;
    const int64_t total_pairs_rows = total_rows > 0 ? total_rows - 1 : 0;
    int nslab = 0, ntasks = 0;
    const size_t pdoubles = gram_partial_doubles(s, 1, &ntasks, &nslab);
    rc = ensure_partial(c, pdoubles);
    if (rc) return rc;
    int64_t chunk = c->chunk_rows;
    if (chunk > (total_pairs_rows + 3) / 4 * 4) chunk = (total_pairs_rows + 3) / 4 * 4;
    if (chunk < 4) chunk = 4;
    const int W = s.width;
    Arena a(c);
    rc = a.reserve(2 * Arena::al((size_t)(chunk + 8) * W * 8) + Arena::al((chunk + 8) * 8) + Arena::al((size_t)(W + 8) * W * 8) + bl.scratch_bytes());
    if (rc) return rc;
// ... 940 lines not shown
```

bluerov2_dynamics_amd/csrc/rollout.hip:

```cpp
#include "brov2_device.h"
#include "brov2_fast.h"
#include "brov2_kernels.h"
#include "brov2_rows.h"

namespace brov {

constexpr int TRIG_REFRESH = 64;

#if BROV_CLOCK_STAMPS
__device__ unsigned long long g_clock_stamps[4096][4];
extern "C" __attribute__((visibility("default"))) int brov_debug_clock_stamps(unsigned long long* host, int nblocks) {
    return (int)hipMemcpyFromSymbol(host, HIP_SYMBOL(g_clock_stamps), sizeof(unsigned long long) * 4 * nblocks, 0, hipMemcpyDeviceToHost);
}
#endif

template <int N>
__device__ __forceinline__ void load_soa(const double* __restrict__ src, int64_t ld, double* r) {
#pragma unroll
    for (int i = 0; i < N; ++i) r[i] = src[i * ld];
}
template <int N>
__device__ __forceinline__ void store_soa(double* __restrict__ dst, int64_t ld, const double* r) {
#pragma unroll
    for (int i = 0; i < N; ++i) dst[i * ld] = r[i];
// ... 181 lines not shown
        for (int i = 0; i < NU; ++i) u[i] = un[i];
        up += (t + 1 < T) ? ustep : 0;
        {
            if constexpr (LAYOUT == LAYOUT_BTU) load_row<NU>(up, un);
            else if constexpr (LAYOUT == LAYOUT_TUB) load_soa<NU>(up, B, un);
            else load_pairs<NU>(up, 2 * B, un);
        }
        step_fast<MODEL, INTEG, LAGMODE, TRACK, GENERIC>(h, p, dt, x, u, lz, Xl, qt, &tcarry, (t & (TRIG_REFRESH - 1)) == 0);
        if (traj && --countdown == 0) {
            countdown = stride;
            store_state();
        }
    }
#if BROV_CLOCK_STAMPS
    if (threadIdx.x == 0 && blockIdx.x < 4096) {
        g_clock_stamps[blockIdx.x][0] = st0; g_clock_stamps[blockIdx.x][1] = sr0;
        g_clock_stamps[blockIdx.x][2] = __builtin_amdgcn_s_memtime(); g_clock_stamps[blockIdx.x][3] = __builtin_amdgcn_s_memrealtime();
    }
#endif
    if (XT) store_row<NX>(XT + b * NX, x);
    if constexpr (MODEL == MODEL_THRUSTER_EULER && TRACK) store_row<24>(lag_io + b * 24, &Xl[0][0]);
}

template <int MODEL, int INTEG, int LAGMODE, bool TRACK>
__global__ void __launch_bounds__(256) rollout_pop_kernel(const FastParams* __restrict__ pg, int64_t B, int64_t T, double dt,
                                                          const double* __restrict__ X0, const double* __restrict__ U, int per_candidate,
                                                          double* __restrict__ lag_io, double* __restrict__ traj, int64_t stride,
                                                          double* __restrict__ XT) {
    constexpr int NX = Dims<MODEL>::NX, NU = Dims<MODEL>::NU;
    __shared__ double2 qt[4];
    init_quadrant_table(qt);
    __syncthreads();
    const int64_t b = (int64_t)blockIdx.x * blockDim.x + threadIdx.x;
    if (b >= B) return;
    const int64_t row = (int64_t)blockIdx.y * B + b;
    const int64_t in = per_candidate ? row : b;
    const CFP p = as_constant(pg + blockIdx.y);
    HotConsts h;
    load_hot(p, h);
    double x[NX];
    load_row<NX>(X0 + in * NX, x);
    LagZ lz;
    double Xl[8][3];
    if constexpr (MODEL == MODEL_THRUSTER_EULER) {
        if constexpr (TRACK) load_row<24>(lag_io + row * 24, &Xl[0][0]);
        else lz.zero();
    }
    double* tp = traj ? traj + row * (T / stride + 1) * NX : nullptr;
    const double* up = U + in * T * NU;
    double un[NU];
    if (T > 0) load_row<NU>(up, un);
    if (traj) { store_row<NX>(tp, x); tp += NX; }
    int64_t countdown = stride;
    for (int64_t t = 0; t < T; ++t) {
        double u[NU];
#pragma unroll
        for (int i = 0; i < NU; ++i) u[i] = un[i];
        up += (t + 1 < T) ? NU : 0;
        load_row<NU>(up, un);
        if constexpr (MODEL == MODEL_THRUSTER_EULER && TRACK) lz.from_thrusters(relaunder(p), Xl);
        step_fast<MODEL, INTEG, LAGMODE, TRACK, true>(h, p, dt, x, u, lz, Xl, qt);
        if (traj && --countdown == 0) {
            countdown = stride;
            store_row<NX>(tp, x);
            tp += NX;
        }
    }
    if (XT) store_row<NX>(XT + row * NX, x);
    if constexpr (MODEL == MODEL_THRUSTER_EULER && TRACK) store_row<24>(lag_io + row * 24, &Xl[0][0]);
}

#ifndef BROV_PAIR_EXP
#define BROV_PAIR_EXP 0
#endif
#ifndef BROV_PAIR_RING
#define BROV_PAIR_RING 2
#endif
#ifndef BROV_PAIR_STAGE
#define BROV_PAIR_STAGE 1
#endif
#ifndef BROV_PAIR_PRIO
#define BROV_PAIR_PRIO 0
#endif
__device__ __forceinline__ void pair_barrier() { asm volatile("s_waitcnt lgkmcnt(0)\n\ts_barrier" ::: "memory"); }

__host__ __device__ constexpr bool pair_saddr_fits(int64_t B) { return B > 0 && B <= (int64_t)((0xFFFFFFFFull - 64 * 16) / (5 * 16)); }
__device__ __forceinline__ uint64_t lane_offset(unsigned& o) { asm volatile("" : "+v"(o)); return o; }
typedef __attribute__((address_space(1))) char* gptr_t;
__device__ __forceinline__ gptr_t wave_uniform(const void* ptr) {
    const uint64_t a = reinterpret_cast<uint64_t>(ptr);
    return (gptr_t)(((uint64_t)(unsigned)__builtin_amdgcn_readfirstlane((int)(a >> 32)) << 32) |
                    (uint64_t)(unsigned)__builtin_amdgcn_readfirstlane((int)(a & 0xFFFFFFFFull)));
}

template <int INTEG, int LAYOUT, int LAGMODE, bool TRACK, bool GENERIC>
__global__ void __launch_bounds__(512) rollout_pair_kernel(const FastParams* __restrict__ pg, int64_t B, int64_t T, double dt,
                                                           const double* __restrict__ X0, const double* __restrict__ U,
                                                           double* __restrict__ lag_io, double* __restrict__ traj,
                                                           int64_t stride, double* __restrict__ XT) {
    constexpr int MODEL = MODEL_THRUSTER_EULER;
    constexpr int NX = 12, NU = 8, NXP = 6, NUP = 4;
    constexpr int NS = (INTEG == INTEG_RK4) ? 4 : 1;
    __shared__ double2 qt[4];
    __shared__ __attribute__((aligned(16))) double2 xch[BROV_PAIR_RING][4][NS * 3][64];
    constexpr bool STG = (LAYOUT == LAYOUT_BTU) && BROV_PAIR_STAGE;
    constexpr int STG_S = 2, STG_ROW = STG_S * NXP + 1, STG_PER = STG_S * NXP;
    __shared__ __attribute__((aligned(16))) double2 stg[STG ? 4 * 64 * STG_ROW : 1];
#if BROV_PAIR_EXP == 4
    __shared__ int pflag[2][4];
    if (threadIdx.x < 8) (&pflag[0][0])[threadIdx.x] = 0;
#endif
    init_quadrant_table(qt);
    __syncthreads();
    const int wave = threadIdx.x >> 6, pair = wave & 3, lane = threadIdx.x & 63;
    const bool thrust = wave >= 4;
#if BROV_PAIR_PRIO
    if (thrust) __builtin_amdgcn_s_setprio(0); else __builtin_amdgcn_s_setprio(3);
#endif
    const int64_t b_raw = (int64_t)blockIdx.x * 256 + pair * 64 + lane;
    const bool live = b_raw < B;
    const int64_t b = live ? b_raw : B - 1;
    const CFP p = as_constant(pg);
    HotConstsResident h;
    load_hot(p, h);

    if (thrust) {
        LagZ lz;
        double Xl[8][3];
        if constexpr (TRACK) { load_row<24>(lag_io + b * 24, &Xl[0][0]); lz.from_thrusters(p, Xl); }
        else lz.zero();
        if constexpr (!GENERIC) lz.to_observer(p);
        const double* up = nullptr;
        int64_t ustep;
        if constexpr (LAYOUT == LAYOUT_BTU) { up = U + b * T * NU; ustep = NU; }
        else if constexpr (LAYOUT == LAYOUT_TUB) { up = U + b; ustep = (int64_t)NU * B; }
        else ustep = (int64_t)NUP * 2 * B;
        const int64_t bw_c = (int64_t)blockIdx.x * 256 + pair * 64 < B ? (int64_t)blockIdx.x * 256 + pair * 64 : B - 1;
        gptr_t ub = LAYOUT == LAYOUT_TPB ? wave_uniform(U + 2 * bw_c) : nullptr;
        unsigned uoff[NUP];
#pragma unroll
        for (int i = 0; i < NUP; ++i) uoff[i] = (unsigned)((b - bw_c) * 16 + (int64_t)i * 16 * B);
        double un[NU];
        int64_t tl = 0;
        auto load_controls = [&]() {
            if constexpr (LAYOUT == LAYOUT_BTU) load_row<NU>(up, un);
            else if constexpr (LAYOUT == LAYOUT_TUB) load_soa<NU>(up, B, un);
            else {
                typedef double v2d __attribute__((ext_vector_type(2)));
#pragma unroll
                for (int i = 0; i < NUP; ++i) {
                    const v2d w = __builtin_nontemporal_load(reinterpret_cast<const __attribute__((address_space(1))) v2d*>(ub + lane_offset(uoff[i])));
                    un[2 * i] = w[0]; un[2 * i + 1] = w[1];
                }
            }
        };
        if (T > 0) load_controls();
        auto produce = [&](int slot) {
            double fcmd[8], acmd[6], a[6];
            const CFP pp = relaunder(p);
            command_accel<MODEL, !GENERIC>(pp, un, fcmd, acmd);
            if constexpr (LAYOUT == LAYOUT_TPB) ub += (tl + 1 != T) ? ustep * 8 : 0;
            else up += (tl + 1 != T) ? ustep : 0;
            ++tl;
            load_controls();
#pragma unroll
            for (int s = 1; s <= NS; ++s) {
                lag_stage_accel<LAGMODE, GENERIC>(h, pp, lz, s, acmd, a);
#pragma unroll
                for (int j = 0; j < 3; ++j) xch[slot][pair][(s - 1) * 3 + j][lane] = make_double2(a[2 * j], a[2 * j + 1]);
            }
            lag_step_advance<INTEG, LAGMODE, TRACK, GENERIC>(relaunder(p), lz, fcmd, acmd, Xl);
        };
#if BROV_PAIR_EXP == 1
        for (int64_t t = 0; t < T; ++t) pair_barrier();
        (void)produce;
#elif BROV_PAIR_EXP == 4
        {
            volatile int* prodf = &pflag[0][pair];
            volatile int* consf = &pflag[1][pair];
            int slot = 0;
            for (int64_t s = 0; s < T; ++s) {
                if (s >= BROV_PAIR_RING) {
                    const int need = (int)(s - BROV_PAIR_RING + 1);
                    int spins = 0;
                    while (*consf < need && ++spins < (1 << 22)) __builtin_amdgcn_s_sleep(1);
                }
                asm volatile("" ::: "memory");
                produce(slot);
                asm volatile("" ::: "memory");
                *prodf = (int)(s + 1);
                slot = (slot + 1 == BROV_PAIR_RING) ? 0 : slot + 1;
            }
        }
#else
        if (T > 0) produce(0);
        for (int64_t t = 1; t < T; ++t) {
            pair_barrier();
            produce((int)(t & 1));
        }
        if (T > 0) pair_barrier();
#endif
        if constexpr (TRACK) { if (live) store_row<24>(lag_io + b * 24, &Xl[0][0]); }
    } else {
        double x[NX];
        load_row<NX>(X0 + b * NX, x);
        double* tp = nullptr;
        int64_t tstep = 0;
        if (traj) {
            if constexpr (LAYOUT == LAYOUT_BTU) { tp = traj + b * (T / stride + 1) * NX; tstep = NX; }
            else if constexpr (LAYOUT == LAYOUT_TUB) { tp = traj + b; tstep = (int64_t)NX * B; }
            else tstep = (int64_t)NXP * 2 * B;
        }
        const int64_t sw_c = (int64_t)blockIdx.x * 256 + pair * 64 < B ? (int64_t)blockIdx.x * 256 + pair * 64 : B - 1;
        gptr_t sb = LAYOUT == LAYOUT_TPB ? wave_uniform(traj + 2 * sw_c) : nullptr;
        unsigned soff[NXP];
#pragma unroll
        for (int i = 0; i < NXP; ++i) soff[i] = (unsigned)((b - sw_c) * 16 + (int64_t)i * 16 * B);
        const bool staged = STG && traj != nullptr && stride == 1 && (uint64_t)(T + 1) * (NX * 8) * 64 < (1ull << 32);
        const int64_t bw = (int64_t)blockIdx.x * 256 + pair * 64;
        constexpr int STG_TPI = 64 / STG_PER, STG_NI = (64 + STG_TPI - 1) / STG_TPI;
        const int st_q = lane / STG_PER, st_c = lane - st_q * STG_PER;
        const unsigned st_rb = (unsigned)((T + 1) * (NX * 8));
        const unsigned st_off = (unsigned)st_q * st_rb + (unsigned)st_c * 16u;
        const int st_lds = st_q * STG_ROW + st_c;
        const int st_live = (int)((B - bw) < 64 ? (B - bw) : 64);
        int st_fill = 0;
        char* st_base = nullptr;
        double2* const st_wave = stg + (STG ? pair * 64 * STG_ROW : 0);
        if constexpr (STG) {
            if (staged) {
                const uint64_t a = reinterpret_cast<uint64_t>(traj) + (uint64_t)bw * (uint64_t)st_rb;
                st_base = reinterpret_cast<char*>(((uint64_t)(unsigned)__builtin_amdgcn_readfirstlane((int)(a >> 32)) << 32) |
                                                  (uint64_t)(unsigned)__builtin_amdgcn_readfirstlane((int)(a & 0xFFFFFFFFull)));
            }
        }
        auto st_flush = [&](int ns) {
            if constexpr (STG) {
                __builtin_amdgcn_wave_barrier();
                asm volatile("s_waitcnt lgkmcnt(0)" ::: "memory");
                if (ns == STG_S) {
#pragma unroll
                    for (int it = 0; it < STG_NI; ++it) {
                        if (lane < STG_TPI * STG_PER && it * STG_TPI + st_q < st_live) {
                            const double2 v = st_wave[st_lds + it * STG_TPI * STG_ROW];
                            *reinterpret_cast<double2*>(st_base + (uint64_t)(it * STG_TPI) * st_rb + st_off) = v;
                        }
                    }
                } else {
                    const int per = ns * NXP;
                    for (int i = lane; i < 64 * per; i += 64) {
                        const int q = i / per, c = i - q * per;
                        const double2 v = st_wave[q * STG_ROW + c];
                        if (q < st_live) *reinterpret_cast<double2*>(st_base + (uint64_t)q * st_rb + (uint64_t)c * 16u) = v;
                    }
                }
                st_base += (int64_t)ns * (NX * 8);
                st_fill = 0;
                __builtin_amdgcn_wave_barrier();
                asm volatile("s_waitcnt lgkmcnt(0)" ::: "memory");
            }
        };
        auto store_state = [&]() {
            if constexpr (STG) {
                if (staged) {
                    double2* row = st_wave + lane * STG_ROW + st_fill * NXP;
#pragma unroll
                    for (int j = 0; j < NXP; ++j) row[j] = make_double2(x[2 * j], x[2 * j + 1]);
                    if (++st_fill == STG_S) st_flush(STG_S);
                    return;
                }
            }
            if constexpr (LAYOUT == LAYOUT_TPB) {
                typedef double v2d __attribute__((ext_vector_type(2)));
#pragma unroll
                for (int i = 0; i < NXP; ++i) {
                    v2d w; w[0] = x[2 * i]; w[1] = x[2 * i + 1];
                    __builtin_nontemporal_store(w, reinterpret_cast<__attribute__((address_space(1))) v2d*>(sb + lane_offset(soff[i])));
                }
                sb += tstep * 8;
                return;
            }
            if (live) {
                if constexpr (LAYOUT == LAYOUT_BTU) store_row<NX>(tp, x);
                else if constexpr (LAYOUT == LAYOUT_TUB) store_soa<NX>(tp, B, x);
            }
            tp += tstep;
        };
        if (traj) store_state();
        int64_t countdown = stride;
        Trig tcarry;
#if BROV_CLOCK_STAMPS
        const unsigned long long st0 = __builtin_amdgcn_s_memtime(), sr0 = __builtin_amdgcn_s_memrealtime();
#endif
#if BROV_PAIR_EXP == 4
        volatile int* prodf = &pflag[0][pair];
        volatile int* consf = &pflag[1][pair];
        int seen = 0, slot = 0;
#endif
        for (int64_t t = 0; t < T; ++t) {
#if BROV_PAIR_EXP == 3
            pair_barrier();
            const double2* src = &xch[t & 1][pair][0][lane];
            if (T >= 0) continue;
#elif BROV_PAIR_EXP == 4
            {
                int spins = 0;
                while (seen < (int)(t + 1) && ++spins < (1 << 22)) { seen = *prodf; if (seen < (int)(t + 1)) __builtin_amdgcn_s_sleep(1); }
            }
            asm volatile("" ::: "memory");
            const double2* src = &xch[slot][pair][0][lane];
            slot = (slot + 1 == BROV_PAIR_RING) ? 0 : slot + 1;
#else
            pair_barrier();
            const double2* src = &xch[t & 1][pair][0][lane];
#endif
            integrate_fast<MODEL, INTEG, GENERIC>(h, p, dt, x, [&](int s, double* a) {
#pragma unroll
                for (int j = 0; j < 3; ++j) { const double2 v = src[((s - 1) * 3 + j) * 64]; a[2 * j] = v.x; a[2 * j + 1] = v.y; }
            }, qt, &tcarry, (t & (TRIG_REFRESH - 1)) == 0);
#if BROV_PAIR_EXP == 4
            asm volatile("" ::: "memory");
            *consf = (int)(t + 1);
            seen = *prodf;
#endif
            if (traj && --countdown == 0) {
                countdown = stride;
                store_state();
            }
        }
#if BROV_CLOCK_STAMPS
        if (wave == 0 && lane == 0 && blockIdx.x < 4096) {
            g_clock_stamps[blockIdx.x][0] = st0; g_clock_stamps[blockIdx.x][1] = sr0;
            g_clock_stamps[blockIdx.x][2] = __builtin_amdgcn_s_memtime(); g_clock_stamps[blockIdx.x][3] = __builtin_amdgcn_s_memrealtime();
        }
#endif
        if constexpr (STG) { if (staged && st_fill > 0) st_flush(st_fill); }
        if (XT && live) store_row<NX>(XT + b * NX, x);
    }
}

constexpr int BTU_TILE = 2;

template <int NU> __device__ __forceinline__ int in_swizzle(int d, int j) {
    if constexpr (NU == 8) return d ^ ((j >> 1) & 7);
    else return d;
}

template <int MODEL, int INTEG, int LAGMODE, bool TRACK, bool GENERIC>
__global__ void __launch_bounds__(256) rollout_btu_lds_kernel(const FastParams* __restrict__ pg, int64_t B, int64_t T, double dt,
                                                              const double* __restrict__ X0, const double* __restrict__ U,
                                                              double* __restrict__ lag_io, double* __restrict__ traj,
                                                              double* __restrict__ XT) {
    constexpr int NX = Dims<MODEL>::NX, NU = Dims<MODEL>::NU;
    constexpr int CH = BTU_TILE * NU / 2;
    constexpr int IN_SLOTS = 64 * CH;
    constexpr int ORS = BTU_TILE * NX + 2;
    constexpr int OCB = (NX % 2 == 0) ? 2 : 1;
    constexpr int OCPR = BTU_TILE * NX / OCB;
    __shared__ __attribute__((aligned(16))) double lds_in[4][2][IN_SLOTS * 2];
    __shared__ __attribute__((aligned(16))) double lds_out[4][64 * ORS];
    __shared__ double2 qt[4];
    init_quadrant_table(qt);
    __syncthreads();

    const int lane = threadIdx.x & 63, wave = threadIdx.x >> 6;
    const int64_t b0w = (int64_t)blockIdx.x * 256 + wave * 64;
    const int64_t b_raw = b0w + lane;
    const bool live = b_raw < B;
    const int64_t b = live ? b_raw : B - 1;
    const CFP p = as_constant(pg);
    HotConsts h;
    load_hot(p, h);
    double x[NX];
    load_row<NX>(X0 + b * NX, x);
    LagZ lz;
    double Xl[8][3];
    if constexpr (MODEL == MODEL_THRUSTER_EULER) {
        if constexpr (TRACK) { load_row<24>(lag_io + b * 24, &Xl[0][0]); lz.from_thrusters(p, Xl); }
        else lz.zero();
        if constexpr (!GENERIC) lz.to_observer(p);
    }
    if (traj && live) store_row<NX>(traj + b * (T + 1) * NX, x);

    auto issue_tile = [&](int64_t k) {
        const int64_t t0 = k * BTU_TILE;
#pragma unroll
        for (int i = 0; i < CH; ++i) {
            const int g = i * 64 + lane;
            const int j = g / CH, c = g % CH;
            const int d = in_swizzle<NU>(c, j);
            int64_t bj = b0w + j;
            if (bj >= B) bj = B - 1;
            int64_t t = t0 + (2 * d) / NU;
            if (t >= T) t = T - 1;
            const double* src = U + (bj * T + t) * NU + (2 * d) % NU;
            __builtin_amdgcn_global_load_lds((const __attribute__((address_space(1))) void*)src,
                                             (__attribute__((address_space(3))) void*)(&lds_in[wave][k & 1][i * 128]), 16, 0, 0);
        }
    };

    const int64_t ntiles = (T + BTU_TILE - 1) / BTU_TILE;
    Trig tcarry;
    if (ntiles > 0) issue_tile(0);
    for (int64_t k = 0; k < ntiles; ++k) {
        __syncthreads();
        if (k + 1 < ntiles) issue_tile(k + 1);
        const double* ib = &lds_in[wave][k & 1][0];
        double* ob = &lds_out[wave][lane * ORS];
        const int64_t t0 = k * BTU_TILE;
#pragma unroll 1
        for (int s = 0; s < BTU_TILE; ++s) {
            if (t0 + s < T) {
                double u[NU];
#pragma unroll
                for (int cc = 0; cc < NU / 2; ++cc) {
                    const int d = s * (NU / 2) + cc;
                    const double2 v = *reinterpret_cast<const double2*>(ib + (lane * CH + in_swizzle<NU>(d, lane)) * 2);
                    u[2 * cc] = v.x; u[2 * cc + 1] = v.y;
                }
                step_fast<MODEL, INTEG, LAGMODE, TRACK, GENERIC>(h, p, dt, x, u, lz, Xl, qt, &tcarry, ((t0 + s) & (TRIG_REFRESH - 1)) == 0);
                if (traj) store_row<NX>(ob + s * NX, x);
            }
// ... 172 lines not shown
#pragma unroll
    for (int i = 0; i < NX; ++i) { const double d = x[i] - ref[i]; e = fma(d, d, e); }
    se[row] = e;
    if (endpoints) store_row<NX>(endpoints + row * NX, x);
    if constexpr (RAGGED) {
        if (target && blockIdx.y == 0) store_row<NX>(target + k * NX, ref);
    }
}

__global__ void __launch_bounds__(1024) sum_kernel(int64_t n, const double* __restrict__ v, double* __restrict__ out) {
    __shared__ double sh[1024];
    const double* vj = v + (int64_t)blockIdx.x * n;
    double a = 0.0;
    for (int64_t i = threadIdx.x; i < n; i += 1024) a += vj[i];
    sh[threadIdx.x] = a;
    __syncthreads();
    for (int s = 512; s > 0; s >>= 1) {
        if ((int)threadIdx.x < s) sh[threadIdx.x] += sh[threadIdx.x + s];
        __syncthreads();
    }
    if (threadIdx.x == 0) out[blockIdx.x] = sh[0];
}

__global__ void __launch_bounds__(256) ensemble_stats_kernel(int64_t P, int64_t M, const double* __restrict__ vals,
                                                             double* __restrict__ out) {
    const int64_t m = (int64_t)blockIdx.x * blockDim.x + threadIdx.x;
    if (m >= M) return;
    const double* v = vals + m;
    double s = 0.0, lo = v[0], hi = lo;
    bool finite = true;
    for (int64_t j = 0; j < P; ++j) {
        const double a = v[j * M];
        finite = finite && isfinite(a);
        s += a;
        lo = a < lo ? a : lo;
        hi = a > hi ? a : hi;
    }
    double mean = s / (double)P;
    double q = 0.0;
    for (int64_t j = 0; j < P; ++j) {
        const double d = v[j * M] - mean;
        q = fma(d, d, q);
    }
    double sd = P > 1 ? sqrt(q / (double)(P - 1)) : 0.0;
    if (!finite) mean = sd = lo = hi = __builtin_nan("");
    out[m] = mean;
    out[M + m] = sd;
    out[2 * M + m] = lo;
    out[3 * M + m] = hi;
}

hipError_t launch_sum(hipStream_t st, int64_t n, const double* v, double* out) {
    hipLaunchKernelGGL(sum_kernel, dim3(1), dim3(1024), 0, st, n, v, out);
    return hipGetLastError();
}
static inline unsigned nblk(int64_t n, int bs) { return (unsigned)((n + bs - 1) / bs); }

#define BROV_LAUNCH_CHECK() do { hipError_t e_ = hipGetLastError(); if (e_ != hipSuccess) return e_; } while (0)

template <int MODEL>
static hipError_t launch_rhs_m(hipStream_t st, const DevParams& p, int64_t B, const double* x, const double* u, double* lag, double* xd,
                               unsigned long long* done, unsigned long long seq) {
    hipLaunchKernelGGL(rhs_kernel<MODEL>, dim3(nblk(B, 256)), dim3(256), 0, st, p, B, x, u, lag, xd, done, seq);
    return hipGetLastError();
}
hipError_t launch_rhs(hipStream_t st, const DevParams& p, int model, int64_t B, const double* x, const double* u, double* lag, double* xd,
                      unsigned long long* done, unsigned long long seq) {
    if (B <= 0) return hipSuccess;
    switch (model) {
        case MODEL_THRUSTER_EULER: return launch_rhs_m<MODEL_THRUSTER_EULER>(st, p, B, x, u, lag, xd, done, seq);
        case MODEL_WRENCH_EULER: return launch_rhs_m<MODEL_WRENCH_EULER>(st, p, B, x, u, lag, xd, done, seq);
        default: return launch_rhs_m<MODEL_WRENCH_QUAT>(st, p, B, x, u, lag, xd, done, seq);
    }
}
hipError_t launch_thruster_forces(hipStream_t st, const DevParams& p, int64_t B, const double* u, double* lag, double* tau,
                                  unsigned long long* done, unsigned long long seq) {
    if (B <= 0) return hipSuccess;
    hipLaunchKernelGGL(thruster_forces_kernel, dim3(nblk(B, 256)), dim3(256), 0, st, p, B, u, lag, tau, done, seq);
    return hipGetLastError();
}

template <int MODEL, int INTEG, int LAYOUT, int LAGMODE, bool TRACK, bool GENERIC>
static hipError_t launch_rollout_g(hipStream_t st, const FastParams* p, int64_t B, int64_t T, double dt, const double* x0,
                                   const double* U, double* lag, double* traj, int64_t stride, double* xT, bool want_lds, bool want_pair) {
    if constexpr (MODEL == MODEL_THRUSTER_EULER) {
        const bool staged_btu = LAYOUT == LAYOUT_BTU && (!traj || stride == 1) && T > 0 && want_lds;
        if (want_pair && !staged_btu && (LAYOUT != LAYOUT_TPB || pair_saddr_fits(B))) {
            hipLaunchKernelGGL((rollout_pair_kernel<INTEG, LAYOUT, LAGMODE, TRACK, GENERIC>), dim3(nblk(B, 256)), dim3(512), 0, st,
                               p, B, T, dt, x0, U, lag, traj, stride, xT);
            return hipGetLastError();
        }
    }
    if (LAYOUT == LAYOUT_BTU && (!traj || stride == 1) && T > 0 && want_lds)
        hipLaunchKernelGGL((rollout_btu_lds_kernel<MODEL, INTEG, LAGMODE, TRACK, GENERIC>), dim3(nblk(B, 256)), dim3(256), 0, st,
                           p, B, T, dt, x0, U, lag, traj, xT);
    else
        hipLaunchKernelGGL((rollout_kernel<MODEL, INTEG, LAYOUT, LAGMODE, TRACK, GENERIC>), dim3(nblk(B, 256)), dim3(256), 0, st,
                           p, B, T, dt, x0, U, lag, traj, stride, xT);
    return hipGetLastError();
}
template <int MODEL, int INTEG, int LAYOUT, int LAGMODE>
static hipError_t launch_rollout_t(hipStream_t st, const FastParams* p, int64_t B, int64_t T, double dt, const double* x0,
                                   const double* U, double* lag, double* traj, int64_t stride, double* xT, int btu_staging) {
    const bool want_lds = (btu_staging & 3) == 1 || ((btu_staging & 3) == 0 && (INTEG == INTEG_EULER || MODEL != MODEL_THRUSTER_EULER));
    const bool generic = (btu_staging & 4) != 0;
    const bool want_pair = (btu_staging & 8) == 0;
    constexpr bool DI = model_is_di(MODEL);
    if (MODEL == MODEL_THRUSTER_EULER && lag) {
        if constexpr (MODEL == MODEL_THRUSTER_EULER) {
            return generic ? launch_rollout_g<MODEL, INTEG, LAYOUT, LAGMODE, true, true>(st, p, B, T, dt, x0, U, lag, traj, stride, xT, want_lds, want_pair)
                           : launch_rollout_g<MODEL, INTEG, LAYOUT, LAGMODE, true, false>(st, p, B, T, dt, x0, U, lag, traj, stride, xT, want_lds, want_pair);
        }
    }
    if (generic && !DI) return launch_rollout_g<MODEL, INTEG, LAYOUT, LAGMODE, false, true>(st, p, B, T, dt, x0, U, lag, traj, stride, xT, want_lds, want_pair);
    return launch_rollout_g<MODEL, INTEG, LAYOUT, LAGMODE, false, false>(st, p, B, T, dt, x0, U, lag, traj, stride, xT, want_lds, want_pair);
}
template <int MODEL, int INTEG, int LAYOUT>
static hipError_t launch_rollout_l(hipStream_t st, const FastParams* p, int lag_mode, int64_t B, int64_t T, double dt,
                                   const double* x0, const double* U, double* lag, double* traj, int64_t stride, double* xT, int btu_staging) {
    if constexpr (MODEL == MODEL_THRUSTER_EULER && INTEG == INTEG_RK4) {
        if (lag_mode == 1) return launch_rollout_t<MODEL, INTEG, LAYOUT, 1>(st, p, B, T, dt, x0, U, lag, traj, stride, xT, btu_staging);
    }
    return launch_rollout_t<MODEL, INTEG, LAYOUT, 0>(st, p, B, T, dt, x0, U, lag, traj, stride, xT, btu_staging);
}
template <int MODEL>
static hipError_t launch_rollout_m(hipStream_t st, const FastParams* p, int integ, int lag_mode, int layout, int64_t B, int64_t T,
                                   double dt, const double* x0, const double* U, double* lag, double* traj, int64_t stride, double* xT, int btu_staging) {
    if (integ == INTEG_EULER) {
        if (layout == LAYOUT_BTU) return launch_rollout_l<MODEL, INTEG_EULER, LAYOUT_BTU>(st, p, lag_mode, B, T, dt, x0, U, lag, traj, stride, xT, btu_staging);
        if (layout == LAYOUT_TUB) return launch_rollout_l<MODEL, INTEG_EULER, LAYOUT_TUB>(st, p, lag_mode, B, T, dt, x0, U, lag, traj, stride, xT, btu_staging);
        return launch_rollout_l<MODEL, INTEG_EULER, LAYOUT_TPB>(st, p, lag_mode, B, T, dt, x0, U, lag, traj, stride, xT, btu_staging);
    }
    if (layout == LAYOUT_BTU) return launch_rollout_l<MODEL, INTEG_RK4, LAYOUT_BTU>(st, p, lag_mode, B, T, dt, x0, U, lag, traj, stride, xT, btu_staging);
    if (layout == LAYOUT_TUB) return launch_rollout_l<MODEL, INTEG_RK4, LAYOUT_TUB>(st, p, lag_mode, B, T, dt, x0, U, lag, traj, stride, xT, btu_staging);
    return launch_rollout_l<MODEL, INTEG_RK4, LAYOUT_TPB>(st, p, lag_mode, B, T, dt, x0, U, lag, traj, stride, xT, btu_staging);
}
hipError_t launch_rollout(hipStream_t st, const FastParams* p, int model, int integ, int lag_mode, int layout, int64_t B, int64_t T,
                          double dt, const double* x0, const double* U, double* lag, double* traj, int64_t stride, double* xT, int btu_staging) {
    if (B <= 0) return hipSuccess;
    switch (model) {
        case MODEL_THRUSTER_EULER: return launch_rollout_m<MODEL_THRUSTER_EULER>(st, p, integ, lag_mode, layout, B, T, dt, x0, U, lag, traj, stride, xT, btu_staging);
        case MODEL_WRENCH_EULER: return launch_rollout_m<MODEL_WRENCH_EULER>(st, p, integ, lag_mode, layout, B, T, dt, x0, U, lag, traj, stride, xT, btu_staging);
        case MODEL_WRENCH_QUAT: return launch_rollout_m<MODEL_WRENCH_QUAT>(st, p, integ, lag_mode, layout, B, T, dt, x0, U, lag, traj, stride, xT, btu_staging);
        case MODEL_DI_THRUSTER_EULER: return launch_rollout_m<MODEL_DI_THRUSTER_EULER>(st, p, integ, lag_mode, layout, B, T, dt, x0, U, nullptr, traj, stride, xT, btu_staging);
        case MODEL_DI_WRENCH_EULER: return launch_rollout_m<MODEL_DI_WRENCH_EULER>(st, p, integ, lag_mode, layout, B, T, dt, x0, U, nullptr, traj, stride, xT, btu_staging);
        default: return launch_rollout_m<MODEL_DI_WRENCH_QUAT>(st, p, integ, lag_mode, layout, B, T, dt, x0, U, nullptr, traj, stride, xT, btu_staging);
    }
}

template <int MODEL, int INTEG, int LAGMODE>
static hipError_t launch_rollout_pop_t(hipStream_t st, const FastParams* p, int P, int per_candidate, int64_t B, int64_t T, double dt,
                                       const double* x0, const double* U, double* lag, double* traj, int64_t stride, double* xT) {
    const int bs = B <= 64 ? 64 : 256;
    const dim3 grid(nblk(B, bs), (unsigned)P);
    if constexpr (MODEL == MODEL_THRUSTER_EULER) {
        if (lag) {
            hipLaunchKernelGGL((rollout_pop_kernel<MODEL, INTEG, LAGMODE, true>), grid, dim3(bs), 0, st, p, B, T, dt, x0, U, per_candidate,
                               lag, traj, stride, xT);
            return hipGetLastError();
        }
    }
    hipLaunchKernelGGL((rollout_pop_kernel<MODEL, INTEG, LAGMODE, false>), grid, dim3(bs), 0, st, p, B, T, dt, x0, U, per_candidate,
                       nullptr, traj, stride, xT);
    return hipGetLastError();
}
template <int MODEL>
static hipError_t launch_rollout_pop_m(hipStream_t st, const FastParams* p, int integ, int lag_mode, int P, int per_candidate, int64_t B,
                                       int64_t T, double dt, const double* x0, const double* U, double* lag, double* traj, int64_t stride,
                                       double* xT) {
    if (integ == INTEG_EULER) return launch_rollout_pop_t<MODEL, INTEG_EULER, 0>(st, p, P, per_candidate, B, T, dt, x0, U, lag, traj, stride, xT);
    if constexpr (MODEL == MODEL_THRUSTER_EULER) {
        if (lag_mode == 1) return launch_rollout_pop_t<MODEL, INTEG_RK4, 1>(st, p, P, per_candidate, B, T, dt, x0, U, lag, traj, stride, xT);
    }
    return launch_rollout_pop_t<MODEL, INTEG_RK4, 0>(st, p, P, per_candidate, B, T, dt, x0, U, lag, traj, stride, xT);
}
hipError_t launch_rollout_pop(hipStream_t st, const FastParams* p, int model, int integ, int lag_mode, int P, int per_candidate, int64_t B,
                              int64_t T, double dt, const double* x0, const double* U, double* lag, double* traj, int64_t stride,
                              double* xT) {
    if (B <= 0 || P <= 0) return hipSuccess;
    switch (model) {
        case MODEL_THRUSTER_EULER: return launch_rollout_pop_m<MODEL_THRUSTER_EULER>(st, p, integ, lag_mode, P, per_candidate, B, T, dt, x0, U, lag, traj, stride, xT);
        case MODEL_WRENCH_EULER: return launch_rollout_pop_m<MODEL_WRENCH_EULER>(st, p, integ, lag_mode, P, per_candidate, B, T, dt, x0, U, nullptr, traj, stride, xT);
        case MODEL_WRENCH_QUAT: return launch_rollout_pop_m<MODEL_WRENCH_QUAT>(st, p, integ, lag_mode, P, per_candidate, B, T, dt, x0, U, nullptr, traj, stride, xT);
        default: return hipErrorInvalidValue;
    }
}

hipError_t launch_ensemble_stats(hipStream_t st, int64_t P, int64_t M, const double* vals, double* out) {
    if (P <= 0 || M <= 0) return hipSuccess;
    hipLaunchKernelGGL(ensemble_stats_kernel, dim3(nblk(M, 256)), dim3(256), 0, st, P, M, vals, out);
    return hipGetLastError();
}

int window_scan_chunk() { return WSCAN_CHUNK; }

template <int NC, bool SEG>
static hipError_t launch_window_lag_scan_n(hipStream_t st, int P, int64_t nwin, const double* d_phi, double* d_rs, double* d_chunk,
                                           const double* d_s0, const unsigned long long* d_wopen) {
    const int64_t nchunks = (nwin + WSCAN_CHUNK - 1) / WSCAN_CHUNK;
    const dim3 gc(nblk(nchunks * NC, 256), (unsigned)P);
    hipLaunchKernelGGL((window_lag_chunk_kernel<NC, SEG>), gc, dim3(256), 0, st, nwin, nchunks, d_phi, d_rs, d_chunk, 0, d_wopen);
    BROV_LAUNCH_CHECK();
    hipLaunchKernelGGL((window_lag_scan_kernel<NC, SEG>), dim3((unsigned)P), dim3(64), 0, st, nchunks, d_phi, d_chunk, d_s0, d_wopen);
    BROV_LAUNCH_CHECK();
    hipLaunchKernelGGL((window_lag_chunk_kernel<NC, SEG>), gc, dim3(256), 0, st, nwin, nchunks, d_phi, d_rs, d_chunk, 1, d_wopen);
    return hipGetLastError();
}
hipError_t launch_window_lag_scan(hipStream_t st, int nc, int P, int64_t nwin, const double* d_phi, double* d_rs, double* d_chunk,
                                  const double* d_s0) {
    if (nwin <= 0 || P <= 0) return hipSuccess;
    return nc == 6 ? launch_window_lag_scan_n<6, false>(st, P, nwin, d_phi, d_rs, d_chunk, d_s0, nullptr)
                   : launch_window_lag_scan_n<8, false>(st, P, nwin, d_phi, d_rs, d_chunk, d_s0, nullptr);
}

template <int MODEL, bool RAGGED>
static hipError_t launch_window_m(hipStream_t st, const FastParams* p, int integ, int P, int64_t nwin, int64_t H, double dt,
                                  const double* X, const double* U, const double* lag_start, double* se, double* endpoints,
                                  const int64_t* wrow, double* target) {
    const dim3 grid(nblk(nwin, 256), (unsigned)P);
    if (integ == INTEG_RK4)
        hipLaunchKernelGGL((window_endpoint_kernel<MODEL, INTEG_RK4, RAGGED>), grid, dim3(256), 0, st, p, nwin, H, dt, X, U, lag_start, se,
                           endpoints, wrow, target);
    else
        hipLaunchKernelGGL((window_endpoint_kernel<MODEL, INTEG_EULER, RAGGED>), grid, dim3(256), 0, st, p, nwin, H, dt, X, U, lag_start, se,
                           endpoints, wrow, target);
    return hipGetLastError();
}

template <bool RAGGED>
// ... 139 lines not shown
```

include/brov2.h:

```cpp
#ifndef BROV2_H
#define BROV2_H

#include <stddef.h>
#include <stdint.h>

#ifdef __cplusplus
extern "C" {
#endif

#define BROV2_ABI_VERSION 1

#if defined(BROV2_BUILDING)
#define BROV_API __attribute__((visibility("default")))
#else
#define BROV_API
#endif

typedef struct brov_ctx brov_ctx;

typedef enum brov_status {
    BROV_OK = 0,
    BROV_ERR_ARG = -1,
    BROV_ERR_HIP = -2,
    BROV_ERR_NOMEM = -3,
    BROV_ERR_NODEVICE = -4,
    BROV_ERR_COMM = -5
} brov_status;

typedef enum brov_model {
    BROV_THRUSTER_EULER = 0, BROV_WRENCH_EULER = 1, BROV_WRENCH_QUAT = 2,
    BROV_DI_THRUSTER_EULER = 3, BROV_DI_WRENCH_EULER = 4, BROV_DI_WRENCH_QUAT = 5
} brov_model;
typedef enum brov_integrator { BROV_EULER = 0, BROV_RK4 = 1 } brov_integrator;
typedef enum brov_lag_mode { BROV_LAG_PER_CALL = 0, BROV_LAG_PER_STEP = 1 } brov_lag_mode;
typedef enum brov_layout { BROV_LAYOUT_BTU = 0, BROV_LAYOUT_TUB = 1, BROV_LAYOUT_TPB = 2 } brov_layout;
typedef enum brov_dist { BROV_DIST_IID_UNIFORM = 0, BROV_DIST_AR1 = 1 } brov_dist;

typedef struct brov_params {
    double rho, g, m, volume;
    double xb, yb, zb;
    double Ix, Iy, Iz;
    double added_mass[6];
    double lin_damp[6];
    double quad_damp[6];
    double current[3];
    double thr_r[8][3];
    double thr_dir[8][3];
    double thrust_poly[5];
    double lag_Ac[9], lag_Bc[3], lag_Cc[3];
} brov_params;

BROV_API int brov_abi_version(void);
BROV_API int brov_create(int device_id, brov_ctx** out);
BROV_API void brov_destroy(brov_ctx* ctx);
BROV_API const char* brov_last_error(const brov_ctx* ctx);
BROV_API int brov_arch_is_supported(const char* gcn_arch_name);
BROV_API int brov_device_arch(const brov_ctx* ctx, char* buf, size_t cap);
BROV_API int brov_xcd_round_robin(const brov_ctx* ctx);
BROV_API int brov_set_stream(brov_ctx* ctx, void* hip_stream);
BROV_API int brov_sync(brov_ctx* ctx);
BROV_API int brov_set_timing(brov_ctx* ctx, int enabled);
BROV_API int brov_last_kernel_ms(brov_ctx* ctx, float* ms);

BROV_API void brov_default_params(brov_params* p);
BROV_API int brov_set_params(brov_ctx* ctx, const brov_params* p);
BROV_API int brov_get_params(const brov_ctx* ctx, brov_params* p);
BROV_API int brov_get_derived(const brov_params* p, double Minv6[6], double alloc6x8[48]);
BROV_API int brov_discretise_lag(const brov_params* p, double dt, double Ad[9], double Bd[3]);

BROV_API int brov_model_nx(int model);
BROV_API int brov_model_nu(int model);

BROV_API int brov_malloc(brov_ctx* ctx, size_t bytes, void** dptr);
BROV_API int brov_free(brov_ctx* ctx, void* dptr);
BROV_API int brov_memcpy_h2d(brov_ctx* ctx, void* dst, const void* src, size_t bytes);
BROV_API int brov_memcpy_d2h(brov_ctx* ctx, void* dst, const void* src, size_t bytes);
BROV_API int brov_memcpy_d2d(brov_ctx* ctx, void* dst, const void* src, size_t bytes);
BROV_API int brov_memset(brov_ctx* ctx, void* dst, int value, size_t bytes);
BROV_API int brov_mem_info(brov_ctx* ctx, size_t* free_bytes, size_t* total_bytes);
BROV_API int brov_upload_bags(brov_ctx* ctx, int64_t nbags, const double* const* bag_ptrs, const int64_t* bag_rows,
                              const int64_t* dst_rows, int cols, double* d_dst);

BROV_API int brov_rhs(brov_ctx* ctx, int model, int64_t B, const double* x, const double* u, double dt,
             double* lag_io, double* xdot);
BROV_API int brov_thruster_forces(brov_ctx* ctx, int64_t B, const double* u, double dt, double* lag_io, double* tau);

BROV_API int brov_rollout(brov_ctx* ctx, int model, int integrator, int lag_mode, int layout,
                 int64_t B, int64_t T, double dt, const double* x0, const double* U,
                 double* lag_io, double* traj, int64_t traj_stride, double* xT);
BROV_API int brov_set_di_gains(brov_ctx* ctx, int nu, const double* K_lin, const double* K_ang);
BROV_API int brov_set_btu_staging(brov_ctx* ctx, int mode);
BROV_API int brov_set_rollout_variant(brov_ctx* ctx, int variant);
BROV_API int brov_rollout_dev(brov_ctx* ctx, int model, int integrator, int lag_mode, int layout,
                     int64_t B, int64_t T, double dt, const double* d_x0, const double* d_U,
                     double* d_lag_io, double* d_traj, int64_t traj_stride, double* d_xT);

BROV_API int brov_window_endpoint_se(brov_ctx* ctx, int model, int integrator, int64_t N, int64_t H, double dt,
                            const double* X, const double* U, int carry_lag,
                            double* se_total, double* per_window);
BROV_API int brov_window_endpoint_se_dev(brov_ctx* ctx, int model, int integrator, int64_t N, int64_t H, double dt,
                                const double* d_X, const double* d_U, int carry_lag,
                                double* d_se_total, double* d_per_window );

BROV_API int brov_window_endpoint_pop(brov_ctx* ctx, int model, int integrator, int64_t P, const brov_params* params ,
                             int64_t N, int64_t H, double dt, const double* X, const double* U, int carry_lag,
                             double* se , double* endpoints );
BROV_API int brov_window_endpoint_pop_dev(brov_ctx* ctx, int model, int integrator, int64_t P, const brov_params* params ,
                                 int64_t N, int64_t H, double dt, const double* d_X, const double* d_U, int carry_lag,
                                 double* d_se , double* d_endpoints );
BROV_API int brov_window_endpoint_pop_ragged(brov_ctx* ctx, int model, int integrator, int64_t P, const brov_params* params ,
                                    int64_t nbags, const int64_t* bag_offsets , int64_t H, double dt,
                                    const double* X, const double* U, int carry_lag, double* se ,
                                    double* endpoints , double* target );
BROV_API int brov_window_endpoint_pop_ragged_dev(brov_ctx* ctx, int model, int integrator, int64_t P, const brov_params* params ,
                                        int64_t nbags, const int64_t* bag_offsets , int64_t H, double dt,
                                        const double* d_X, const double* d_U, int carry_lag, double* d_se ,
                                        double* d_endpoints , double* d_target ,
                                        double* d_per_window );
BROV_API int brov_window_endpoint_se_ragged(brov_ctx* ctx, int model, int integrator, int64_t nbags,
                                   const int64_t* bag_offsets , int64_t H, double dt, const double* X,
                                   const double* U, int carry_lag, double* se_total, double* per_window);
BROV_API int brov_window_endpoint_se_ragged_dev(brov_ctx* ctx, int model, int integrator, int64_t nbags,
                                       const int64_t* bag_offsets , int64_t H, double dt, const double* d_X,
                                       const double* d_U, int carry_lag, double* d_se_total, double* d_per_window );
BROV_API int brov_fd_normal_eq_dev(brov_ctx* ctx, int nx, int m, int64_t W, const double* d_endpoints, const double* d_target,
                          const double* delta_host, const double* weight_host, double* JtJ_host, double* Jtr_host);

BROV_API int brov_rollout_pop(brov_ctx* ctx, int model, int integrator, int lag_mode, int64_t P, const brov_params* params ,
                     int inputs_per_candidate, int64_t B, int64_t T, double dt, const double* x0, const double* U,
                     double* lag_io, double* traj, int64_t traj_stride, double* xT);
BROV_API int brov_rollout_pop_dev(brov_ctx* ctx, int model, int integrator, int lag_mode, int64_t P, const brov_params* params ,
                         int inputs_per_candidate, int64_t B, int64_t T, double dt, const double* d_x0, const double* d_U,
                         double* d_lag_io, double* d_traj, int64_t traj_stride, double* d_xT);
BROV_API int brov_ensemble_stats_dev(brov_ctx* ctx, int64_t P, int64_t M, const double* d_vals, double* d_out);

typedef struct brov_feedback {
    double K[8][12], Ki[8][6];
    double u_min[8], u_max[8];
    double z_max[6];
    int32_t hold, _pad;
} brov_feedback;
BROV_API int brov_rollout_feedback(brov_ctx* ctx, int model, int integrator, int lag_mode, int64_t P, const brov_params* params ,
                          int64_t nfb, const brov_feedback* fb , int inputs_per_candidate, int64_t B, int64_t T,
                          double dt, const double* x0, const double* u_ff, const double* ref, int64_t ref_rows, double* lag_io,
                          double* z_io, double* traj, int64_t traj_stride, double* xT, double* u_applied, double* metrics);
BROV_API int brov_rollout_feedback_dev(brov_ctx* ctx, int model, int integrator, int lag_mode, int64_t P, const brov_params* params ,
                              int64_t nfb, const brov_feedback* fb , int inputs_per_candidate, int64_t B, int64_t T,
                              double dt, const double* d_x0, const double* d_u_ff, const double* d_ref, int64_t ref_rows,
                              double* d_lag_io, double* d_z_io, double* d_traj, int64_t traj_stride, double* d_xT,
                              double* d_u_applied, double* d_metrics);

typedef struct brov_ukf {
    double q[12];
    double r[12];
    double alpha, beta, kappa;
} brov_ukf;
BROV_API int brov_ukf_filter(brov_ctx* ctx, int model, int integrator, int lag_mode, int64_t P, const brov_params* params ,
                    int64_t nrec, const brov_ukf* ukf , int64_t B, int64_t T, double dt, const double* x0,
                    const double* P0, const double* U, const double* Y, double* lag_io, double* xf, double* pstd, double* innov,
                    double* xT, double* PT, double* info);
BROV_API int brov_ukf_filter_dev(brov_ctx* ctx, int model, int integrator, int lag_mode, int64_t P, const brov_params* params ,
                        int64_t nrec, const brov_ukf* ukf , int64_t B, int64_t T, double dt, const double* d_x0,
                        const double* d_P0, const double* d_U, const double* d_Y, double* d_lag_io, double* d_xf, double* d_pstd,
                        double* d_innov, double* d_xT, double* d_PT, double* d_info);

BROV_API int brov_ukf_filter_tape_dev(brov_ctx* ctx, int model, int integrator, int lag_mode, int64_t P, const brov_params* params ,
                             int64_t nrec, const brov_ukf* ukf , int64_t B, int64_t T, double dt, const double* d_x0,
                             const double* d_P0, const double* d_U, const double* d_Y, double* d_lag_io, double* d_xf, double* d_pstd,
                             double* d_innov, double* d_xT, double* d_PT, double* d_info, double* d_tape, double* d_nrows);
BROV_API int brov_ukf_rts_dev(brov_ctx* ctx, int64_t P, int64_t B, int64_t T, const double* d_xf, const double* d_tape, const double* d_nrows,
                     const double* d_xs_T, const double* d_Ps_T, double* d_xs, double* d_pstd_s, double* d_Ps, double* d_Ps0,
                     double* d_sinfo);
BROV_API int brov_ukf_smooth(brov_ctx* ctx, int model, int integrator, int lag_mode, int64_t P, const brov_params* params ,
                    int64_t nrec, const brov_ukf* ukf , int64_t B, int64_t T, double dt, const double* x0,
                    const double* P0, const double* U, const double* Y, double* lag_io, double* xf, double* pstd, double* innov,
// ... 177 lines not shown
```

Before: 28.00 billion steps/s.

## Speculate rare-branch-free RK4 step in pair kernel, redo step on rare events

Adds a speculative RK4 step form for the thruster-Euler pair rollout kernel. Rare paths (trig range extension, cos(theta) clamp) are not taken inline; instead, wave ballots record whether any lane would need them, and the step is recomputed with the plain form when that happens. The aim is to strip divergent rare branches and their register pressure from the hot loop. The cost is an extra step recomputation whenever a rare condition fires, plus more template complexity and optional device counters.

```diff
diff --git a/bluerov2_dynamics_amd/_lib.py b/bluerov2_dynamics_amd/_lib.py
--- a/bluerov2_dynamics_amd/_lib.py
+++ b/bluerov2_dynamics_amd/_lib.py
@@ -266,6 +266,7 @@
     "edmdc_set_kmeans_bounds_rate": (ctypes.c_int, [c_void_p, ctypes.c_double]),
     "brov_experiments_build": (ctypes.c_int, []),
     "brov_set_rollout_variant": (ctypes.c_int, [c_void_p, ctypes.c_int]),
+    "brov_set_rollout_spec": (ctypes.c_int, [c_void_p, ctypes.c_int, c_void_p]),
     "edmdc_set_kmeans_far_select": (ctypes.c_int, [c_void_p, c_void_p, c_void_p]),
     "edmdc_kmeans_relocations": (ctypes.c_int, [c_void_p]),
     "edmdc_kmeans_loop_info": (ctypes.c_int, [c_void_p, ctypes.POINTER(ctypes.c_int)]),
@@ -465,6 +466,9 @@
     def set_rollout_variant(self, variant: int):
         self.check(self.lib.brov_set_rollout_variant(self.h, int(variant)), "brov_set_rollout_variant")
 
+    def set_rollout_spec(self, plain_form: bool = False, counts_ptr=None):
+        self.check(self.lib.brov_set_rollout_spec(self.h, int(bool(plain_form)), c_void_p(counts_ptr or 0)), "brov_set_rollout_spec")
+
     def set_kmeans_far_select(self, numpy_rule: bool):
         fn = ctypes.cast(_NUMPY_FAR_SELECT, c_void_p) if numpy_rule else None
         self.check(self.lib.edmdc_set_kmeans_far_select(self.h, fn, None), "edmdc_set_kmeans_far_select")
diff --git a/bluerov2_dynamics_amd/csrc/brov2_fast.h b/bluerov2_dynamics_amd/csrc/brov2_fast.h
--- a/bluerov2_dynamics_amd/csrc/brov2_fast.h
+++ b/bluerov2_dynamics_amd/csrc/brov2_fast.h
@@ -44,6 +44,13 @@
 #endif
 #ifndef BROV_PSI_FRAME
 #define BROV_PSI_FRAME 1
+#endif
+#ifndef BROV_SPEC_CEILING
+#if defined(BROV_PAIR_EXP) && BROV_PAIR_EXP == 5
+#define BROV_SPEC_CEILING 1
+#else
+#define BROV_SPEC_CEILING 0
+#endif
 #endif
 #define BROV_PIN_V(x) asm volatile("" : "+v"(x))
 #define BROV_PIN_S(x) asm volatile("" : "+s"(x))
@@ -121,8 +128,10 @@
     sincos_fast(ang[2], t.spsi, t.cpsi, qt, kv);
 }
 
-template <bool SHORT = false, bool LEAN = false>
-__device__ __forceinline__ void trig_delta(const Trig& b, double d[3], Trig& t, double* dpsi = nullptr, const double* kv = nullptr) {
+template <bool SHORT = false, bool LEAN = false, bool SPEC = false>
+__device__ __forceinline__ void trig_delta(const Trig& b, double d[3], Trig& t, double* dpsi = nullptr, const double* kv = nullptr,
+                                           unsigned long long* rare = nullptr) {
+    static_assert(!SPEC || LEAN, "the speculative form exists for the LEAN kernels only");
     constexpr int K0 = SHORT ? 4 : 3;
     const double S7 = kv ? kv[0] : -1.98412698298579493134e-04, C8 = kv ? kv[1] : 2.48015872894767294178e-05;
     double dcopy[3] = {d[0], d[1], d[2]};
@@ -130,7 +139,8 @@
     int k = 0;
     const double m = fmax(fmax(fabs(d[0]), fabs(d[1])), fabs(d[2]));
     const bool far = !(m <= (SHORT ? 0.0625 : 0.125));
-    if (far) {
+    if constexpr (SPEC) *rare |= __builtin_amdgcn_ballot_w64(far);
+    else if (far) {
         double mf = m;
         if constexpr (LEAN) asm volatile("; trig_delta range extension, rare" : "+v"(mf));
         int e;
@@ -172,7 +182,8 @@
             }
         }
     };
-    if constexpr (LEAN) {
+    if constexpr (SPEC) (void)doubling;
+    else if constexpr (LEAN) {
         if (far) {
             double mf = m;
             asm volatile("; trig_delta doubling, rare" : "+v"(mf));
@@ -234,8 +245,9 @@
     out[0] = o0; out[1] = o1; out[2] = o2; out[3] = o3; out[4] = o4; out[5] = o5;
 }
 
-template <bool GENERIC, class HC, bool PFRAME = false>
-__device__ __forceinline__ void rhs_fast_euler(const HC& h, CFP p, const double x[12], const double a[6], double xd[12], const Trig& tg) {
+template <bool GENERIC, class HC, bool PFRAME = false, bool SPEC = false>
+__device__ __forceinline__ void rhs_fast_euler(const HC& h, CFP p, const double x[12], const double a[6], double xd[12], const Trig& tg,
+                                               unsigned long long* rare = nullptr) {
     const double sphi = tg.sphi, cphi = tg.cphi, sth = tg.sth, cth = tg.cth, spsi = tg.spsi, cpsi = tg.cpsi;
     const double* nu = x + 6;
     const double ctsp = cth * sphi, ctcp = cth * cphi;
@@ -261,7 +273,8 @@
     }
 #if BROV_CLAMP_BRANCH
     double ic = recip_fast(cth);
-    if (__builtin_amdgcn_ballot_w64(fabs(cth) < 1e-7) != 0) {
+    if constexpr (SPEC) *rare |= __builtin_amdgcn_ballot_w64(fabs(cth) < 1e-7);
+    else if (__builtin_amdgcn_ballot_w64(fabs(cth) < 1e-7) != 0) {
         asm volatile("; cos(theta) clamp, rare" ::: "memory");
         if (fabs(cth) < 1e-7) ic = recip_fast(1e-7 * ((cth > 0.0) - (cth < 0.0)));
     }
@@ -329,12 +342,13 @@
     for (int i = 0; i < 6; ++i) xd[7 + i] = a[i];
 }
 
-template <int MODEL, bool GENERIC, class HC, bool PFRAME = false>
-__device__ __forceinline__ void rhs_fast(const HC& h, CFP p, const double* x, const double a[6], double* xd, const Trig& tg) {
+template <int MODEL, bool GENERIC, class HC, bool PFRAME = false, bool SPEC = false>
+__device__ __forceinline__ void rhs_fast(const HC& h, CFP p, const double* x, const double a[6], double* xd, const Trig& tg,
+                                         unsigned long long* rare = nullptr) {
     if constexpr (MODEL == MODEL_DI_WRENCH_QUAT) rhs_di_quat(x, a, xd);
     else if constexpr (model_is_di(MODEL)) rhs_di_euler(x, a, xd, tg);
     else if constexpr (MODEL == MODEL_WRENCH_QUAT) rhs_fast_quat<GENERIC>(h, p, x, a, xd);
-    else rhs_fast_euler<GENERIC, HC, PFRAME>(h, p, x, a, xd, tg);
+    else rhs_fast_euler<GENERIC, HC, PFRAME, SPEC>(h, p, x, a, xd, tg, rare);
 }
 
 struct LagZ {
@@ -461,12 +475,19 @@
     }
 }
 
-template <int MODEL, int INTEG, bool GENERIC, class HC, class AccelFn>
-__device__ __forceinline__ void integrate_fast(const HC& h, CFP p, double dt, double* x, AccelFn&& accel,
-                                               const double2* qt, Trig* carry, bool refresh) {
+template <class Fn> struct SpecStep { Fn committed; };
+template <class Fn> __device__ __forceinline__ SpecStep<Fn> spec_step(Fn fn) { return SpecStep<Fn>{fn}; }
+template <class T> struct is_spec_step : std::false_type {};
+template <class Fn> struct is_spec_step<SpecStep<Fn>> : std::true_type {};
+template <int MODEL, int INTEG, bool GENERIC, class HC, class AccelFn, class Form = std::nullptr_t>
+__device__ __forceinline__ unsigned long long integrate_fast(const HC& h, CFP p, double dt, double* x, AccelFn&& accel,
+                                               const double2* qt, Trig* carry, bool refresh, Form form = nullptr) {
+    constexpr bool SPEC = is_spec_step<Form>::value;
     constexpr int NX = Dims<MODEL>::NX;
     constexpr bool ANG = !model_is_quat(MODEL);
     constexpr bool LEAN = HC::RESIDENT && !GENERIC;
+    static_assert(!SPEC || (LEAN && INTEG == INTEG_RK4 && MODEL == MODEL_THRUSTER_EULER), "speculative step: RK4 body wave of the reference vehicle only");
+    unsigned long long rare = 0;
     double a[6];
     Trig tb, ts;
     const bool CARRY = ANG && carry != nullptr;
@@ -504,7 +525,7 @@
                 if (ANG && i >= 3 && i < 6) dl[i - 3] = c * k[i];
                 else xs[i] = fma(c, k[i], x[i]);
             }
-            if constexpr (ANG) trig_delta<BROV_TRIG_SHORT && decltype(HALF)::value, LEAN>(tb, dl, ts, PSIF ? dps : nullptr, trig_consts<GENERIC>(h));
+            if constexpr (ANG) trig_delta<BROV_TRIG_SHORT && decltype(HALF)::value, LEAN, SPEC>(tb, dl, ts, PSIF ? dps : nullptr, trig_consts<GENERIC>(h), &rare);
         };
         auto add_turned = [&](double w) {
             const double r0 = fma(dps[1], k[0], fma(-dps[0], k[1], k[0])), r1 = fma(dps[0], k[0], fma(dps[1], k[1], k[1]));
@@ -512,24 +533,44 @@
             xn[1] = fma(w, r1, xn[1]);
         };
         accel(1, a);
-        rhs_fast<MODEL, GENERIC, HC, PSIF>(h, p, x, a, k, tb);
+        rhs_fast<MODEL, GENERIC, HC, PSIF, SPEC>(h, p, x, a, k, tb, &rare);
 #pragma unroll
         for (int i = 0; i < NX; ++i) xn[i] = ((CARRY && i >= 3 && i < 6) || (PSIF && i < 2)) ? h6 * k[i] : fma(h6, k[i], x[i]);
         stage_state(h2, std::true_type{});
         accel(2, a);
-        rhs_fast<MODEL, GENERIC, HC, PSIF>(h, p, xs, a, k, ts);
+        rhs_fast<MODEL, GENERIC, HC, PSIF, SPEC>(h, p, xs, a, k, ts, &rare);
 #pragma unroll
         for (int i = PSIF ? 2 : 0; i < NX; ++i) xn[i] = fma(h3, k[i], xn[i]);
         if constexpr (PSIF) add_turned(h3);
         stage_state(h2, std::true_type{});
         accel(3, a);
-        rhs_fast<MODEL, GENERIC, HC, PSIF>(h, p, xs, a, k, ts);
+        rhs_fast<MODEL, GENERIC, HC, PSIF, SPEC>(h, p, xs, a, k, ts, &rare);
 #pragma unroll
         for (int i = PSIF ? 2 : 0; i < NX; ++i) xn[i] = fma(h3, k[i], xn[i]);
         if constexpr (PSIF) add_turned(h3);
         stage_state(dt, std::false_type{});
         accel(4, a);
-        rhs_fast<MODEL, GENERIC, HC, PSIF>(h, p, xs, a, k, ts);
+        rhs_fast<MODEL, GENERIC, HC, PSIF, SPEC>(h, p, xs, a, k, ts, &rare);
+        if constexpr (SPEC) {
+            add_turned(h6);
+#pragma unroll
+            for (int i = 3; i < 6; ++i) dang[i - 3] = fma(h6, k[i], xn[i]);
+            rare |= __builtin_amdgcn_ballot_w64(!(fmax(fmax(fabs(dang[0]), fabs(dang[1])), fabs(dang[2])) <= 0.125));
+#if !BROV_SPEC_CEILING
+            if (rare != 0) return rare;
+#endif
+            x[0] = fma(tb.cpsi, xn[0], fma(-tb.spsi, xn[1], x[0]));
+            x[1] = fma(tb.spsi, xn[0], fma(tb.cpsi, xn[1], x[1]));
+#pragma unroll
+            for (int i = 2; i < NX; ++i) {
+                if (i >= 3 && i < 6) { x[i] += dang[i - 3]; BROV_FORM_HERE(x[i]); }
+                else x[i] = fma(h6, k[i], xn[i]);
+            }
+            unsigned long long decided = 0;
+            trig_delta<false, LEAN, true>(tb, dang, *carry, nullptr, trig_consts<GENERIC>(h), &decided);
+            form.committed();
+            return 0;
+        }
         if constexpr (PSIF) {
             add_turned(h6);
             x[0] = fma(tb.cpsi, xn[0], fma(-tb.spsi, xn[1], x[0]));
@@ -548,6 +589,7 @@
     }
     if constexpr (ANG) { if (CARRY) trig_delta<false, LEAN>(tb, dang, *carry, nullptr, trig_consts<GENERIC>(h)); }
     if constexpr (model_is_quat(MODEL)) quat_normalize(x + 3);
+    return 0;
 }
 
 template <int INTEG, int LAGMODE, bool TRACK, bool GENERIC>
diff --git a/bluerov2_dynamics_amd/csrc/brov2_kernels.h b/bluerov2_dynamics_amd/csrc/brov2_kernels.h
--- a/bluerov2_dynamics_amd/csrc/brov2_kernels.h
+++ b/bluerov2_dynamics_amd/csrc/brov2_kernels.h
@@ -12,7 +12,7 @@
                                   unsigned long long* done = nullptr, unsigned long long seq = 0);
 hipError_t launch_rollout(hipStream_t st, const FastParams* d_fp, int model, int integ, int lag_mode, int layout, int64_t B,
                           int64_t T, double dt, const double* x0, const double* U, double* lag, double* traj,
-                          int64_t stride, double* xT, int btu_staging);
+                          int64_t stride, double* xT, int btu_staging, unsigned long long* spec_counts = nullptr);
 hipError_t launch_rollout_pop(hipStream_t st, const FastParams* d_fp, int model, int integ, int lag_mode, int P, int per_candidate,
                               int64_t B, int64_t T, double dt, const double* x0, const double* U, double* lag, double* traj,
                               int64_t stride, double* xT);
diff --git a/bluerov2_dynamics_amd/csrc/capi.hip b/bluerov2_dynamics_amd/csrc/capi.hip
--- a/bluerov2_dynamics_amd/csrc/capi.hip
+++ b/bluerov2_dynamics_amd/csrc/capi.hip
@@ -46,6 +46,8 @@
     brov_pinc_hyper train_hyper = {};
     int btu_staging = 0;
     int single_lane = 0;
+    int pair_plain = 0;
+    unsigned long long* spec_counts = nullptr;
     int64_t chunk_rows = (int64_t)1 << 20;
     char* lift_cache = nullptr;
     size_t lift_cache_cap = 0;
@@ -1111,7 +1113,7 @@
     HIPCK(c, launch_rollout(c->stream, model_is_di_h(model) ? c->d_fp_di : c->d_fp, model, integ, lag_mode, layout, B, T, dt, d_x0, d_U,
                             d_lag_io, d_traj, d_traj ? stride : 1, d_xT,
                             c->btu_staging | ((c->fp.has_current || c->fp.has_xy || c->fp.tm_dense || c->fp.obs_bad) ? 4 : 0) |
-                                (c->single_lane ? 8 : 0)));
+                                (c->single_lane ? 8 : 0) | (c->pair_plain ? 16 : 0), c->spec_counts));
     return BROV_OK;
 }
 
@@ -2554,6 +2556,12 @@
 int brov_set_rollout_variant(brov_ctx* c, int variant) {
     if (!c || variant < 0 || variant > 1) return fail(c, BROV_ERR_ARG, "brov_set_rollout_variant: variant must be 0 or 1");
     c->single_lane = variant;
+    return BROV_OK;
+}
+int brov_set_rollout_spec(brov_ctx* c, int plain_form, unsigned long long* d_counts) {
+    if (!c || plain_form < 0 || plain_form > 1) return fail(c, BROV_ERR_ARG, "brov_set_rollout_spec: plain_form must be 0 or 1");
+    c->pair_plain = plain_form;
+    c->spec_counts = d_counts;
     return BROV_OK;
 }
 int brov_experiments_build(void) {
diff --git a/bluerov2_dynamics_amd/csrc/rollout.hip b/bluerov2_dynamics_amd/csrc/rollout.hip
--- a/bluerov2_dynamics_amd/csrc/rollout.hip
+++ b/bluerov2_dynamics_amd/csrc/rollout.hip
@@ -287,6 +287,11 @@
 #ifndef BROV_PAIR_PRIO
 #define BROV_PAIR_PRIO 0
 #endif
+#if BROV_PAIR_EXP == 5
+template <bool ON> __device__ __forceinline__ auto ceiling_tag() { if constexpr (ON) return spec_step([]() {}); else return nullptr; }
+#else
+template <bool ON> __device__ __forceinline__ std::nullptr_t ceiling_tag() { return nullptr; }
+#endif
 __device__ __forceinline__ void pair_barrier() { asm volatile("s_waitcnt lgkmcnt(0)\n\ts_barrier" ::: "memory"); }
 
 __host__ __device__ constexpr bool pair_saddr_fits(int64_t B) { return B > 0 && B <= (int64_t)((0xFFFFFFFFull - 64 * 16) / (5 * 16)); }
@@ -298,11 +303,11 @@
                     (uint64_t)(unsigned)__builtin_amdgcn_readfirstlane((int)(a & 0xFFFFFFFFull)));
 }
 
-template <int INTEG, int LAYOUT, int LAGMODE, bool TRACK, bool GENERIC>
-__global__ void __launch_bounds__(512) rollout_pair_kernel(const FastParams* __restrict__ pg, int64_t B, int64_t T, double dt,
-                                                           const double* __restrict__ X0, const double* __restrict__ U,
-                                                           double* __restrict__ lag_io, double* __restrict__ traj,
-                                                           int64_t stride, double* __restrict__ XT) {
+template <int INTEG, int LAYOUT, int LAGMODE, bool TRACK, bool GENERIC, bool SPEC>
+__device__ __forceinline__ void pair_rollout(const FastParams* __restrict__ pg, int64_t B, int64_t T, double dt,
+                                             const double* __restrict__ X0, const double* __restrict__ U,
+                                             double* __restrict__ lag_io, double* __restrict__ traj,
+                                             int64_t stride, double* __restrict__ XT, unsigned long long* __restrict__ counts) {
     constexpr int MODEL = MODEL_THRUSTER_EULER;
     constexpr int NX = 12, NU = 8, NXP = 6, NUP = 4;
     constexpr int NS = (INTEG == INTEG_RK4) ? 4 : 1;
@@ -465,7 +470,7 @@
                 asm volatile("s_waitcnt lgkmcnt(0)" ::: "memory");
             }
         };
-        auto store_state = [&]() {
+        auto store_state = [&](auto HOT) {
             if constexpr (STG) {
                 if (staged) {
                     double2* row = st_wave + lane * STG_ROW + st_fill * NXP;
@@ -480,7 +485,8 @@
 #pragma unroll
                 for (int i = 0; i < NXP; ++i) {
                     v2d w; w[0] = x[2 * i]; w[1] = x[2 * i + 1];
-                    __builtin_nontemporal_store(w, reinterpret_cast<__attribute__((address_space(1))) v2d*>(sb + lane_offset(soff[i])));
+                    const uint64_t o = decltype(HOT)::value ? lane_offset(soff[i]) : (uint64_t)soff[i];
+                    __builtin_nontemporal_store(w, reinterpret_cast<__attribute__((address_space(1))) v2d*>(sb + o));
                 }
                 sb += tstep * 8;
                 return;
@@ -491,7 +497,7 @@
             }
             tp += tstep;
         };
-        if (traj) store_state();
+        if (traj) store_state(std::true_type{});
         int64_t countdown = stride;
         Trig tcarry;
 #if BROV_CLOCK_STAMPS
@@ -502,6 +508,53 @@
         volatile int* consf = &pflag[1][pair];
         int seen = 0, slot = 0;
 #endif
+        if constexpr (SPEC) {
+            const double2* src = nullptr;
+            auto accel = [&](int s, double* a) {
+#pragma unroll
+                for (int j = 0; j < 3; ++j) { const double2 v = src[((s - 1) * 3 + j) * 64]; a[2 * j] = v.x; a[2 * j + 1] = v.y; }
+            };
+            if (!traj) countdown = INT64_MAX;
+            auto stored = [&](auto HOT) {
+                if (--countdown == 0) {
+                    countdown = stride;
+                    store_state(HOT);
+                }
+            };
+            unsigned long long n_redo = 0, n_plain = 0;
+            const int64_t Tn = T > 0 ? T : 0;
+            int64_t t = 0;
+            while (t != Tn) {
+                trig_full(x + 3, tcarry, qt, trig_consts<GENERIC>(h));
+                unsigned long long rare;
+                do {
+                    pair_barrier();
+                    src = &xch[t & 1][pair][0][lane];
+                    rare = integrate_fast<MODEL, INTEG, GENERIC>(h, p, dt, x, accel, qt, &tcarry, false, spec_step([&]() {
+                        stored(std::true_type{});
+                        ++t;
+                    }));
+                } while (!((rare != 0) | ((t & (TRIG_REFRESH - 1)) == 0) | (t == Tn)));
+                if (rare != 0) {
+                    integrate_fast<MODEL, INTEG, GENERIC>(h, p, dt, x, accel, qt, &tcarry, false);
+                    stored(std::false_type{});
+                    ++t;
+                    ++n_redo;
+                    while ((t & (TRIG_REFRESH - 1)) != 0 && t != Tn) {
+                        pair_barrier();
+                        src = &xch[t & 1][pair][0][lane];
+                        integrate_fast<MODEL, INTEG, GENERIC>(h, p, dt, x, accel, qt, &tcarry, false);
+                        stored(std::false_type{});
+                        ++t;
+                        ++n_plain;
+                    }
+                }
+            }
+            if (counts != nullptr && lane == 0) {
+                unsigned long long* c = counts + ((int64_t)blockIdx.x * 4 + pair) * 2;
+                c[0] = n_redo; c[1] = n_plain;
+            }
+        } else
         for (int64_t t = 0; t < T; ++t) {
 #if BROV_PAIR_EXP == 3
             pair_barrier();
@@ -522,7 +575,7 @@
             integrate_fast<MODEL, INTEG, GENERIC>(h, p, dt, x, [&](int s, double* a) {
 #pragma unroll
                 for (int j = 0; j < 3; ++j) { const double2 v = src[((s - 1) * 3 + j) * 64]; a[2 * j] = v.x; a[2 * j + 1] = v.y; }
-            }, qt, &tcarry, (t & (TRIG_REFRESH - 1)) == 0);
+            }, qt, &tcarry, (t & (TRIG_REFRESH - 1)) == 0, ceiling_tag<INTEG == INTEG_RK4 && !GENERIC>());
 #if BROV_PAIR_EXP == 4
             asm volatile("" ::: "memory");
             *consf = (int)(t + 1);
@@ -530,7 +583,7 @@
 #endif
             if (traj && --countdown == 0) {
                 countdown = stride;
-                store_state();
+                store_state(std::true_type{});
             }
         }
 #if BROV_CLOCK_STAMPS
@@ -543,6 +596,23 @@
         if (XT && live) store_row<NX>(XT + b * NX, x);
     }
 }
+
+template <int INTEG, int LAYOUT, int LAGMODE, bool TRACK, bool GENERIC>
+__global__ void __launch_bounds__(512) rollout_pair_kernel(const FastParams* __restrict__ pg, int64_t B, int64_t T, double dt,
+                                                           const double* __restrict__ X0, const double* __restrict__ U,
+                                                           double* __restrict__ lag_io, double* __restrict__ traj,
+                                                           int64_t stride, double* __restrict__ XT) {
+    pair_rollout<INTEG, LAYOUT, LAGMODE, TRACK, GENERIC, false>(pg, B, T, dt, X0, U, lag_io, traj, stride, XT, nullptr);
+}
+
+template <int LAYOUT, int LAGMODE, bool TRACK>
+__global__ void __launch_bounds__(512) rollout_spec_kernel(const FastParams* __restrict__ pg, int64_t B, int64_t T, double dt,
+                                                           const double* __restrict__ X0, const double* __restrict__ U,
+                                                           double* __restrict__ lag_io, double* __restrict__ traj,
+                                                           int64_t stride, double* __restrict__ XT, unsigned long long* __restrict__ counts) {
+    pair_rollout<INTEG_RK4, LAYOUT, LAGMODE, TRACK, false, true>(pg, B, T, dt, X0, U, lag_io, traj, stride, XT, counts);
+}
+constexpr bool spec_layout(int layout) { return layout == LAYOUT_TPB; }
 
 constexpr int BTU_TILE = 2;
 
@@ -881,10 +951,18 @@
 
 template <int MODEL, int INTEG, int LAYOUT, int LAGMODE, bool TRACK, bool GENERIC>
 static hipError_t launch_rollout_g(hipStream_t st, const FastParams* p, int64_t B, int64_t T, double dt, const double* x0,
-                                   const double* U, double* lag, double* traj, int64_t stride, double* xT, bool want_lds, bool want_pair) {
+                                   const double* U, double* lag, double* traj, int64_t stride, double* xT, bool want_lds, bool want_pair,
+                                   bool want_spec, unsigned long long* spec_counts) {
     if constexpr (MODEL == MODEL_THRUSTER_EULER) {
         const bool staged_btu = LAYOUT == LAYOUT_BTU && (!traj || stride == 1) && T > 0 && want_lds;
         if (want_pair && !staged_btu && (LAYOUT != LAYOUT_TPB || pair_saddr_fits(B))) {
+            if constexpr (INTEG == INTEG_RK4 && !GENERIC && spec_layout(LAYOUT)) {
+                if (want_spec) {
+                    hipLaunchKernelGGL((rollout_spec_kernel<LAYOUT, LAGMODE, TRACK>), dim3(nblk(B, 256)), dim3(512), 0, st,
+                                       p, B, T, dt, x0, U, lag, traj, stride, xT, spec_counts);
+                    return hipGetLastError();
+                }
+            }
             hipLaunchKernelGGL((rollout_pair_kernel<INTEG, LAYOUT, LAGMODE, TRACK, GENERIC>), dim3(nblk(B, 256)), dim3(512), 0, st,
                                p, B, T, dt, x0, U, lag, traj, stride, xT);
             return hipGetLastError();
@@ -900,50 +978,55 @@
 }
 template <int MODEL, int INTEG, int LAYOUT, int LAGMODE>
 static hipError_t launch_rollout_t(hipStream_t st, const FastParams* p, int64_t B, int64_t T, double dt, const double* x0,
-                                   const double* U, double* lag, double* traj, int64_t stride, double* xT, int btu_staging) {
+                                   const double* U, double* lag, double* traj, int64_t stride, double* xT, int btu_staging,
+                                   unsigned long long* spec_counts) {
     const bool want_lds = (btu_staging & 3) == 1 || ((btu_staging & 3) == 0 && (INTEG == INTEG_EULER || MODEL != MODEL_THRUSTER_EULER));
     const bool generic = (btu_staging & 4) != 0;
     const bool want_pair = (btu_staging & 8) == 0;
+    const bool want_spec = (btu_staging & 16) == 0;
     constexpr bool DI = model_is_di(MODEL);
     if (MODEL == MODEL_THRUSTER_EULER && lag) {
         if constexpr (MODEL == MODEL_THRUSTER_EULER) {
-            return generic ? launch_rollout_g<MODEL, INTEG, LAYOUT, LAGMODE, true, true>(st, p, B, T, dt, x0, U, lag, traj, stride, xT, want_lds, want_pair)
-                           : launch_rollout_g<MODEL, INTEG, LAYOUT, LAGMODE, true, false>(st, p, B, T, dt, x0, U, lag, traj, stride, xT, want_lds, want_pair);
-        }
-    }
-    if (generic && !DI) return launch_rollout_g<MODEL, INTEG, LAYOUT, LAGMODE, false, true>(st, p, B, T, dt, x0, U, lag, traj, stride, xT, want_lds, want_pair);
-    return launch_rollout_g<MODEL, INTEG, LAYOUT, LAGMODE, false, false>(st, p, B, T, dt, x0, U, lag, traj, stride, xT, want_lds, want_pair);
+            return generic ? launch_rollout_g<MODEL, INTEG, LAYOUT, LAGMODE, true, true>(st, p, B, T, dt, x0, U, lag, traj, stride, xT, want_lds, want_pair, want_spec, spec_counts)
+                           : launch_rollout_g<MODEL, INTEG, LAYOUT, LAGMODE, true, false>(st, p, B, T, dt, x0, U, lag, traj, stride, xT, want_lds, want_pair, want_spec, spec_counts);
+        }
+    }
+    if (generic && !DI) return launch_rollout_g<MODEL, INTEG, LAYOUT, LAGMODE, false, true>(st, p, B, T, dt, x0, U, lag, traj, stride, xT, want_lds, want_pair, want_spec, spec_counts);
+    return launch_rollout_g<MODEL, INTEG, LAYOUT, LAGMODE, false, false>(st, p, B, T, dt, x0, U, lag, traj, stride, xT, want_lds, want_pair, want_spec, spec_counts);
 }
 template <int MODEL, int INTEG, int LAYOUT>
 static hipError_t launch_rollout_l(hipStream_t st, const FastParams* p, int lag_mode, int64_t B, int64_t T, double dt,
-                                   const double* x0, const double* U, double* lag, double* traj, int64_t stride, double* xT, int btu_staging) {
+                                   const double* x0, const double* U, double* lag, double* traj, int64_t stride, double* xT, int btu_staging,
+                                   unsigned long long* spec_counts) {
     if constexpr (MODEL == MODEL_THRUSTER_EULER && INTEG == INTEG_RK4) {
-        if (lag_mode == 1) return launch_rollout_t<MODEL, INTEG, LAYOUT, 1>(st, p, B, T, dt, x0, U, lag, traj, stride, xT, btu_staging);
-    }
-    return launch_rollout_t<MODEL, INTEG, LAYOUT, 0>(st, p, B, T, dt, x0, U, lag, traj, stride, xT, btu_staging);
+        if (lag_mode == 1) return launch_rollout_t<MODEL, INTEG, LAYOUT, 1>(st, p, B, T, dt, x0, U, lag, traj, stride, xT, btu_staging, spec_counts);
+    }
+    return launch_rollout_t<MODEL, INTEG, LAYOUT, 0>(st, p, B, T, dt, x0, U, lag, traj, stride, xT, btu_staging, spec_counts);
 }
 template <int MODEL>
 static hipError_t launch_rollout_m(hipStream_t st, const FastParams* p, int integ, int lag_mode, int layout, int64_t B, int64_t T,
-                                   double dt, const double* x0, const double* U, double* lag, double* traj, int64_t stride, double* xT, int btu_staging) {
+                                   double dt, const double* x0, const double* U, double* lag, double* traj, int64_t stride, double* xT, int btu_staging,
+                                   unsigned long long* spec_counts) {
     if (integ == INTEG_EULER) {
-        if (layout == LAYOUT_BTU) return launch_rollout_l<MODEL, INTEG_EULER, LAYOUT_BTU>(st, p, lag_mode, B, T, dt, x0, U, lag, traj, stride, xT, btu_staging);
-        if (layout == LAYOUT_TUB) return launch_rollout_l<MODEL, INTEG_EULER, LAYOUT_TUB>(st, p, lag_mode, B, T, dt, x0, U, lag, traj, stride, xT, btu_staging);
-        return launch_rollout_l<MODEL, INTEG_EULER, LAYOUT_TPB>(st, p, lag_mode, B, T, dt, x0, U, lag, traj, stride, xT, btu_staging);
-    }
-    if (layout == LAYOUT_BTU) return launch_rollout_l<MODEL, INTEG_RK4, LAYOUT_BTU>(st, p, lag_mode, B, T, dt, x0, U, lag, traj, stride, xT, btu_staging);
-    if (layout == LAYOUT_TUB) return launch_rollout_l<MODEL, INTEG_RK4, LAYOUT_TUB>(st, p, lag_mode, B, T, dt, x0, U, lag, traj, stride, xT, btu_staging);
-    return launch_rollout_l<MODEL, INTEG_RK4, LAYOUT_TPB>(st, p, lag_mode, B, T, dt, x0, U, lag, traj, stride, xT, btu_staging);
+        if (layout == LAYOUT_BTU) return launch_rollout_l<MODEL, INTEG_EULER, LAYOUT_BTU>(st, p, lag_mode, B, T, dt, x0, U, lag, traj, stride, xT, btu_staging, spec_counts);
+        if (layout == LAYOUT_TUB) return launch_rollout_l<MODEL, INTEG_EULER, LAYOUT_TUB>(st, p, lag_mode, B, T, dt, x0, U, lag, traj, stride, xT, btu_staging, spec_counts);
+        return launch_rollout_l<MODEL, INTEG_EULER, LAYOUT_TPB>(st, p, lag_mode, B, T, dt, x0, U, lag, traj, stride, xT, btu_staging, spec_counts);
+    }
+    if (layout == LAYOUT_BTU) return launch_rollout_l<MODEL, INTEG_RK4, LAYOUT_BTU>(st, p, lag_mode, B, T, dt, x0, U, lag, traj, stride, xT, btu_staging, spec_counts);
+    if (layout == LAYOUT_TUB) return launch_rollout_l<MODEL, INTEG_RK4, LAYOUT_TUB>(st, p, lag_mode, B, T, dt, x0, U, lag, traj, stride, xT, btu_staging, spec_counts);
+    return launch_rollout_l<MODEL, INTEG_RK4, LAYOUT_TPB>(st, p, lag_mode, B, T, dt, x0, U, lag, traj, stride, xT, btu_staging, spec_counts);
 }
 hipError_t launch_rollout(hipStream_t st, const FastParams* p, int model, int integ, int lag_mode, int layout, int64_t B, int64_t T,
-                          double dt, const double* x0, const double* U, double* lag, double* traj, int64_t stride, double* xT, int btu_staging) {
+                          double dt, const double* x0, const double* U, double* lag, double* traj, int64_t stride, double* xT, int btu_staging,
+                                   unsigned long long* spec_counts) {
     if (B <= 0) return hipSuccess;
     switch (model) {
-        case MODEL_THRUSTER_EULER: return launch_rollout_m<MODEL_THRUSTER_EULER>(st, p, integ, lag_mode, layout, B, T, dt, x0, U, lag, traj, stride, xT, btu_staging);
-        case MODEL_WRENCH_EULER: return launch_rollout_m<MODEL_WRENCH_EULER>(st, p, integ, lag_mode, layout, B, T, dt, x0, U, lag, traj, stride, xT, btu_staging);
-        case MODEL_WRENCH_QUAT: return launch_rollout_m<MODEL_WRENCH_QUAT>(st, p, integ, lag_mode, layout, B, T, dt, x0, U, lag, traj, stride, xT, btu_staging);
-        case MODEL_DI_THRUSTER_EULER: return launch_rollout_m<MODEL_DI_THRUSTER_EULER>(st, p, integ, lag_mode, layout, B, T, dt, x0, U, nullptr, traj, stride, xT, btu_staging);
-        case MODEL_DI_WRENCH_EULER: return launch_rollout_m<MODEL_DI_WRENCH_EULER>(st, p, integ, lag_mode, layout, B, T, dt, x0, U, nullptr, traj, stride, xT, btu_staging);
-        default: return launch_rollout_m<MODEL_DI_WRENCH_QUAT>(st, p, integ, lag_mode, layout, B, T, dt, x0, U, nullptr, traj, stride, xT, btu_staging);
+        case MODEL_THRUSTER_EULER: return launch_rollout_m<MODEL_THRUSTER_EULER>(st, p, integ, lag_mode, layout, B, T, dt, x0, U, lag, traj, stride, xT, btu_staging, spec_counts);
+        case MODEL_WRENCH_EULER: return launch_rollout_m<MODEL_WRENCH_EULER>(st, p, integ, lag_mode, layout, B, T, dt, x0, U, lag, traj, stride, xT, btu_staging, spec_counts);
+        case MODEL_WRENCH_QUAT: return launch_rollout_m<MODEL_WRENCH_QUAT>(st, p, integ, lag_mode, layout, B, T, dt, x0, U, lag, traj, stride, xT, btu_staging, spec_counts);
+        case MODEL_DI_THRUSTER_EULER: return launch_rollout_m<MODEL_DI_THRUSTER_EULER>(st, p, integ, lag_mode, layout, B, T, dt, x0, U, nullptr, traj, stride, xT, btu_staging, spec_counts);
+        case MODEL_DI_WRENCH_EULER: return launch_rollout_m<MODEL_DI_WRENCH_EULER>(st, p, integ, lag_mode, layout, B, T, dt, x0, U, nullptr, traj, stride, xT, btu_staging, spec_counts);
+        default: return launch_rollout_m<MODEL_DI_WRENCH_QUAT>(st, p, integ, lag_mode, layout, B, T, dt, x0, U, nullptr, traj, stride, xT, btu_staging, spec_counts);
     }
 }
 
diff --git a/include/brov2.h b/include/brov2.h
--- a/include/brov2.h
+++ b/include/brov2.h
@@ -91,6 +91,7 @@
 BROV_API int brov_set_di_gains(brov_ctx* ctx, int nu, const double* K_lin, const double* K_ang);
 BROV_API int brov_set_btu_staging(brov_ctx* ctx, int mode);
 BROV_API int brov_set_rollout_variant(brov_ctx* ctx, int variant);
+BROV_API int brov_set_rollout_spec(brov_ctx* ctx, int plain_form, unsigned long long* d_counts);
 BROV_API int brov_rollout_dev(brov_ctx* ctx, int model, int integrator, int lag_mode, int layout,
                      int64_t B, int64_t T, double dt, const double* d_x0, const double* d_U,
                      double* d_lag_io, double* d_traj, int64_t traj_stride, double* d_xT);
```

Result: slower. 27.16 billion steps/s (-3.0%).
